# TRIQS/maxent

Hardware: AMD Instinct MI355X
Metric: alpha-solves/s (higher is better)
Workload: dtype f64; 1 GPU; cfg4: ElementwiseMaxEnt 16x16 G(tau) = 256 alpha scans x 100 alpha = 25600 alpha-solves, n_tau=200 n_omega=500 n_s=56; the one batch sharded over 1 GPU(s), element e on rank e mod N; in_flight=1, step=chain kernel + device line fit, problems_on_rank0=25600, kernel=mxe::chain_kernel_mc<32, 2>, waves_per_chain=4, workgroups=512, lds_bytes=77824

## Files before the change

### maxent_amd/csrc/maxent_hip.hip

```cpp
#include "../../include/maxent_hip.h"
#include "mxe_kernel.hip.h"
#include "mxe_kernel_mc.hip.h"
#include "mxe_kernel_lv.hip.h"
#include "mxe_eval.hip.h"
#include "mxe_plan.h"

#include <algorithm>
#include <chrono>
#include <cmath>
#include <cstdio>
#include <cstdlib>
#include <cstring>
#include <new>
#include <string>
#include <map>
#include <vector>
#include <mutex>
#include <thread>
#include <tuple>

using mxe::KParams;

namespace {

// ... 141 lines not shown
            while ((e = hipEventQuery(g_pinned.ev[j & 1])) == hipErrorNotReady) {}
            if (e == hipSuccess) std::memcpy((char*)dst + j * C, g_pinned.buf[j & 1], len);
        }
    }
    return e;
}

template <typename T> struct DevBuf {
    T* p = nullptr; size_t n = 0;
    size_t bytes = 0;
    hipError_t ensure(size_t count) {
        if (count <= n && p) return hipSuccess;
        const size_t need = std::max<size_t>(count, 1) * sizeof(T);
        if (p && need <= bytes) { n = count; return hipSuccess; }
        if (p) { hipDeviceSynchronize(); release(); }
        size_t got = 0;
        void* q = g_pool.take(need, &got);
        static const bool poison = getenv("MXE_POISON_ALLOC") != nullptr;
        if (q) { p = (T*)q; bytes = got; n = count; if (poison) { hipMemset(p, 0xA5, bytes); hipDeviceSynchronize(); } return hipSuccess; }
        hipError_t e = hipMalloc((void**)&p, need);
        if (e == hipSuccess) { n = count; bytes = need; if (poison) { hipMemset(p, 0xA5, bytes); hipDeviceSynchronize(); } }
        return e;
    }
    void release() { if (p && !g_pool.give(p, bytes)) hipFree(p); p = nullptr; n = 0; bytes = 0; }
};

}

struct mxe_ctx {
    int device = 0, n_cu = 256;
    hipStream_t stream = nullptr;
    hipEvent_t ev0 = nullptr, ev1 = nullptr, ev_mark = nullptr;
    int n_tau = 0, n_omega = 0, n_s = 0, NP = 64, nwp = 0;
    std::vector<double> U, S, V;
    std::vector<DataSet> ds;
    bool ds_dirty = true;
    int n_elem = 0;
    std::vector<int> elem_ds, elem_kind;
    std::vector<double> h_sumD, h_D;
    int n_chain = 0, n_alpha = 0;
    std::vector<int> chain_elem;
    std::vector<int> sub_elem, sub_prob0, sub_len, sub_v0, wg_chains;
    int n_sub = 0, n_wg = 0, mc_na = 0, mc_wgpc = 1, wgpc_auto = 2, n_queue = 0, n_solo = 0;
    std::vector<int> excluded;
    DevBuf<int> dexcluded;
    bool mc_gst = false;
    int lv_mode = 0;
    int mc_wgpc_hint = 1;
    int n_wg2 = 0, wgpc2 = 1;
    DevBuf<int> d2_elem, d2_prob0, d2_len, d2_v0, d2_queue, dcnt1_niter, dcnt1_nevals;
    DevBuf<int> drounds;
    int rounds_n[2] = {0, 0};
    int placement_checked = 0;
    DevBuf<double> dgstate_mc;
    std::vector<int> queue;
    std::vector<int> sub_pre;
    std::vector<int> sub_walk0;
    std::vector<double> walk_alpha;
    bool has_walk = false;
    bool has_pre = false;
    mxe_opts opts;
    bool chains_ready = false, launched = false;
    int last_nw = 0, last_lds = 0;
    std::string last_kernel;
    DevBuf<float> dVf, dVtf;
    DevBuf<double> dsel3;
    std::vector<double> h_sel3;
    double* pre_d = nullptr; int32_t* pre_i = nullptr; bool pre_scaled = false;
    double* pre_rows = nullptr; int pre_first = 0, pre_count = 0; bool pre_index = false;
    double* h_sel3_pinned = nullptr; size_t h_sel3_pinned_n = 0;
    DevBuf<double> dproj_U, dproj_err, dproj_G;
    DevBuf<long long> dproj_off;
    bool proj_ready = false;
    std::vector<double> h_rperp;
    std::vector<long long> elem_roff;
    DevBuf<double> drperp;
    DevBuf<long long> delem_roff;
    bool rperp_dirty = false, roff_ready = false;
    DevBuf<double> dV, dVx, dVt, dc, dcinv, dghat, dcperp, dD, dsumD, dalpha, dv0;
    DevBuf<int> delem_ds, delem_kind, dchain_elem, dsub_prob0, dsub_len, dsub_v0, dwg_chains;
    DevBuf<double> dout_v, dout_pack, dout_pack2, dB, dA, dlogdet;
    DevBuf<int> dparent_elem;
    int result_buffer = 0;
    struct View { double* p = nullptr; } dout_H, dout_chi2, dout_S, dout_Q;
    DevBuf<int> dout_niter, dout_nact;
    struct IView { int* p = nullptr; } dout_conv, dout_nevals;
    DevBuf<long long> dprof;
    DevBuf<int> dqueue, dcounter;
    DevBuf<int> dsub_pre, dsub_init, dsub_walk0;
    DevBuf<double> dwalk_alpha;
    DevBuf<double> dinit_tab;
    DevBuf<double> dgstate;
    DevBuf<int> dfin_budget, dfin_out;
    DevBuf<double> dfin_alpha;
    DevBuf<int> dfin_elem, dfin_prob0, dfin_len, dfin_v0;
    DevBuf<double> dfin_start;
    int sel3_nc = 0;
    int last_finished = 0;
    int last_rungs = 0;
    bool has_init = false;
    DevBuf<double> ev_x, ev_alpha, ev_scal, ev_vecw, ev_vecs, ev_mat;
    DevBuf<int> ev_elem;
    DevBuf<double> pv_d;
    DevBuf<int> pv_i;
    DevBuf<double> ps_d;
    DevBuf<double> rr_d;
    DevBuf<int> rr_i;
    DevBuf<double> er_d;
    DevBuf<int> er_i;
    DevBuf<long long> er_l;
    DevBuf<double> rows_out;
    DevBuf<int> rows_idx;
    double chi2_factor = 1.0;
    struct mxe_comm_state* comm = nullptr;
    std::string hip_err;
};

#define MXE_CATCH_ALL \
    catch (const std::bad_alloc&) { return MXE_ERR_NOMEM; } \
    catch (...) { return MXE_ERR_ARG; }

#define HIPCHK(ctx, call) do { hipError_t e__ = (call); if (e__ != hipSuccess) { \
    (ctx)->hip_err = std::string(#call) + ": " + hipGetErrorString(e__); return MXE_ERR_HIP; } } while (0)

namespace {

void jacobi_svd(std::vector<double>& C, int m, int n, std::vector<double>& Q)
{
    Q.assign((size_t)n * n, 0.0);
    for (int i = 0; i < n; ++i) Q[(size_t)i * n + i] = 1.0;
    const double eps = 2.220446049250313e-16;
    for (int sweep = 0; sweep < 60; ++sweep) {
        bool rotated = false;
        for (int p = 0; p < n - 1; ++p) {
            for (int q = p + 1; q < n; ++q) {
                double a = 0.0, b = 0.0, g = 0.0;
                for (int i = 0; i < m; ++i) {
                    const double x = C[(size_t)i * n + p], y = C[(size_t)i * n + q];
                    a += x * x; b += y * y; g += x * y;
                }
                if (a == 0.0 || b == 0.0) continue;
                if (std::fabs(g) <= eps * std::sqrt(a * b)) continue;
                rotated = true;
                const double zeta = (b - a) / (2.0 * g);
                const double t = (zeta >= 0 ? 1.0 : -1.0) /
                                 (std::fabs(zeta) + std::sqrt(1.0 + zeta * zeta));
                const double cs = 1.0 / std::sqrt(1.0 + t * t), sn = cs * t;
                for (int i = 0; i < m; ++i) {
                    const double x = C[(size_t)i * n + p], y = C[(size_t)i * n + q];
                    C[(size_t)i * n + p] = cs * x - sn * y;
                    C[(size_t)i * n + q] = sn * x + cs * y;
                }
                for (int i = 0; i < n; ++i) {
                    const double x = Q[(size_t)i * n + p], y = Q[(size_t)i * n + q];
                    Q[(size_t)i * n + p] = cs * x - sn * y;
                    Q[(size_t)i * n + q] = sn * x + cs * y;
                }
            }
        }
        if (!rotated) break;
    }
}

int build_dataset(mxe_ctx* ctx, int n_rows, const double* U_rot, const double* err, DataSet& d)
{
    const int ns = ctx->n_s;
// ... 588 lines not shown
int g_placement[MXE_MAX_DEVICES];
std::mutex g_placement_mu;

int placement_rule_holds(mxe_ctx* ctx, int n_cu, bool* holds)
{
    *holds = false;
    if (getenv("MXE_FORCE_NO_SOLO_RULE")) return MXE_OK;
    const int dev = ctx->device;
    if (dev < 0 || dev >= MXE_MAX_DEVICES) return MXE_OK;
    std::lock_guard<std::mutex> lk(g_placement_mu);
    if (g_placement[dev] == 0) {
        const int n = 2 * n_cu;
        DevBuf<unsigned> d;
        HIPCHK(ctx, d.ensure((size_t)2 * n));
        HIPCHK(ctx, hipFuncSetAttribute((const void*)placement_probe_kernel, hipFuncAttributeMaxDynamicSharedMemorySize, 73728));
        std::vector<unsigned> h((size_t)2 * n);
        bool ok = true;
        for (int rep = 0; rep < 2 && ok; ++rep) {
            hipLaunchKernelGGL(placement_probe_kernel, dim3(n), dim3(256), 73728, ctx->stream, d.p);
            HIPCHK(ctx, hipGetLastError());
            HIPCHK(ctx, hipMemcpyAsync(h.data(), d.p, h.size() * 4, hipMemcpyDeviceToHost, ctx->stream));
            HIPCHK(ctx, stream_wait(ctx->stream));
            for (int b = 0; b < n_cu && ok; ++b)
                ok = ((h[2 * b] >> 8) & 0xff) == ((h[2 * (b + n_cu)] >> 8) & 0xff) && (h[2 * b + 1] & 0xf) == (h[2 * (b + n_cu) + 1] & 0xf);
        }
        d.release();
        g_placement[dev] = ok ? 1 : 2;
    }
    *holds = g_placement[dev] == 1;
    return MXE_OK;
}

void read_plan_env(mxe::PlanEnv& env)
{
    if (const char* e = getenv("MXE_TAPER")) env.taper = std::max(0.2, atof(e));
    if (const char* e = getenv("MXE_LADDER_RATIO")) env.ladder_ratio = std::max(1.05, atof(e));
    env.no_lds_basis = getenv("MXE_NO_LDS_BASIS") != nullptr; env.no_split_by_kind = getenv("MXE_NO_SPLIT_BY_KIND") != nullptr;
    env.no_ladder = getenv("MXE_NO_LADDER") != nullptr; env.no_na64 = getenv("MXE_NO_NA64") != nullptr; env.no_sorted_static = getenv("MXE_NO_SORTED_STATIC") != nullptr;
}
}

int mxe_chains_upload(mxe_ctx* ctx, int n_chain, int n_alpha,
                      const int32_t* elem_of_chain, const double* alpha_scaled,
                      const double* v0, const mxe_opts* opts)
try {
    if (!ctx || n_chain < 1 || n_alpha < 1 || !elem_of_chain || !alpha_scaled || !v0) return MXE_ERR_ARG;
    if (ctx->n_elem < 1) return MXE_ERR_STATE;
    HIPCHK(ctx, hipSetDevice(ctx->device));
    if (ctx->ds_dirty) { int rc = upload_bases(ctx); if (rc != MXE_OK) return rc; }
    const int ns = ctx->n_s, NP = ctx->NP, nw = ctx->n_omega, nwp = ctx->nwp;
    const size_t P = (size_t)n_chain * n_alpha;
    mxe_opts o; if (opts) o = *opts; else mxe_opts_default(&o);
    if (o.maxiter < 1 || o.step_max <= 0 || o.mu_first <= 0 || o.mu_grow <= 1.0 || o.decouple_tol < 0) return MXE_ERR_ARG;
    if (o.waves_per_chain != 0 && o.waves_per_chain != 1 && o.waves_per_chain != 2 && o.waves_per_chain != 4 && o.waves_per_chain != 8) return MXE_ERR_ARG;
    if (o.chains_per_wg != 0 && o.chains_per_wg != 1 && o.chains_per_wg != 4) return MXE_ERR_ARG;
    if (o.alpha_split < 0 || o.wg_per_cu < 0 || o.wg_per_cu > 2 || o.in_flight < 0 || o.in_flight > 64) return MXE_ERR_ARG;
    if (o.precision != MXE_PRECISION_F64 && o.precision != MXE_PRECISION_F32) return MXE_ERR_ARG;
    if (o.precision == MXE_PRECISION_F32 && NP != 64) return MXE_ERR_LIMIT;
    if (!(o.chi2_factor > 0.0) || !std::isfinite(o.chi2_factor)) return MXE_ERR_ARG;
    for (int c = 0; c < n_chain; ++c) if (elem_of_chain[c] < 0 || elem_of_chain[c] >= ctx->n_elem) return MXE_ERR_ARG;
    for (size_t i = 0; i < P; ++i) if (!(alpha_scaled[i] > 0.0) || !std::isfinite(alpha_scaled[i])) return MXE_ERR_ARG;
    std::vector<double> hv0((size_t)n_chain * NP, 0.0);
    for (int c = 0; c < n_chain; ++c) {
        const DataSet& DS = ctx->ds[ctx->elem_ds[elem_of_chain[c]]];
        for (int k = 0; k < ns; ++k) {
            double s = DS.identity_q ? v0[(size_t)c * ns + k] : 0.0;
            if (!DS.identity_q) for (int j = 0; j < ns; ++j) s += DS.Q[(size_t)j * ns + k] * v0[(size_t)c * ns + j];
            hv0[(size_t)c * NP + k] = s;
        }
    }
    std::vector<double> alpha_dev(alpha_scaled, alpha_scaled + P);
    if (o.chi2_factor != 1.0) for (double& a : alpha_dev) a /= o.chi2_factor;
    std::vector<int> ds_rows(ctx->ds.size()); std::vector<double> ds_c32(ctx->ds.size(), 0.0);
    for (size_t d = 0; d < ctx->ds.size(); ++d) { ds_rows[d] = ctx->ds[d].n_rows; if (ns > 32) ds_c32[d] = ctx->ds[d].c[32]; }
    mxe::PlanInput in;
    in.n_chain = n_chain; in.n_alpha = n_alpha; in.elem_of_chain = elem_of_chain; in.alpha = alpha_dev.data();
    in.elem_kind = ctx->elem_kind.data(); in.elem_ds = ctx->elem_ds.data(); in.elem_sumD = ctx->h_sumD.data();
    in.n_ds = (int)ctx->ds.size(); in.ds_rows = ds_rows.data(); in.ds_c32 = ds_c32.data();
    in.n_s = ns; in.NP = NP; in.n_omega_pad = nwp; in.n_cu = ctx->n_cu; in.opts = o;
    in.lds_lv = mxe::lv_lds_bytes(ns, nwp) + mxe::LV_STATIC_LDS; in.lds_mc64x1 = mc_lds_bytes(64, nwp, 1);
    in.lds_mc32x1 = mc_lds_bytes(32, nwp, 1); in.lds_mc32x2 = mc_lds_bytes(32, nwp, 2);
    in.wgpc_auto = ctx->wgpc_auto; in.mc_wgpc_hint = ctx->mc_wgpc_hint;
    read_plan_env(in.env);
    mxe::LaunchPlan plan;
    if (const int rc = mxe::plan_launch(in, plan); rc != MXE_OK) {
        if (plan.uncovered || plan.covered_twice) fprintf(stderr, "mxe_chains_upload: %zu problems covered by no piece, %zu by two (layout %d, %zu pieces, %zu excluded)\n",
                                                          plan.uncovered, plan.covered_twice, plan.layout, plan.pieces.size(), plan.excluded.size());
        return rc;
    }
    int n_solo = 0, placement_checked = 0;
    if (plan.solo_rule) {
        bool holds = false;
        if (plan.n_solo_wanted > 0) { const int rp = placement_rule_holds(ctx, ctx->n_cu, &holds); if (rp != MXE_OK) return rp; }
        placement_checked = holds ? 1 : 2; n_solo = (holds && plan.lv_mode != 2) ? plan.n_solo_wanted : 0;
    }
    ctx->chains_ready = false; ctx->launched = false; ctx->sel3_nc = 0; ctx->has_init = false;
    ctx->opts = o; ctx->opts.precision = plan.precision; ctx->chi2_factor = o.chi2_factor;
    ctx->n_chain = n_chain; ctx->n_alpha = n_alpha; ctx->chain_elem.assign(elem_of_chain, elem_of_chain + n_chain);
    const size_t n_sub = plan.pieces.size();
    for (auto* v : {&ctx->sub_elem, &ctx->sub_prob0, &ctx->sub_len, &ctx->sub_v0, &ctx->sub_pre, &ctx->sub_walk0}) v->resize(n_sub);
    ctx->n_sub = (int)n_sub; ctx->has_pre = false;
    for (size_t sc = 0; sc < n_sub; ++sc) {
        const mxe::Piece& p = plan.pieces[sc];
        ctx->sub_elem[sc] = p.elem; ctx->sub_prob0[sc] = p.prob0; ctx->sub_len[sc] = p.len; ctx->sub_v0[sc] = p.v0;
        ctx->sub_pre[sc] = p.pre; ctx->sub_walk0[sc] = p.walk0; ctx->has_pre |= p.pre > 0;
    }
    ctx->has_walk = !plan.walk_alpha.empty(); ctx->walk_alpha = std::move(plan.walk_alpha); ctx->excluded = std::move(plan.excluded);
    ctx->queue = std::move(plan.queue); ctx->wg_chains = std::move(plan.wg_chains); ctx->n_queue = (int)ctx->queue.size();
    ctx->mc_na = plan.mc_na; ctx->mc_wgpc = plan.mc_wgpc; ctx->mc_gst = plan.mc_gst; ctx->lv_mode = plan.lv_mode;
    ctx->wgpc_auto = plan.wgpc_auto; ctx->mc_wgpc_hint = plan.mc_wgpc_hint; ctx->n_wg = plan.n_wg; ctx->n_wg2 = plan.n_wg2; ctx->wgpc2 = plan.wgpc2;
    ctx->n_solo = n_solo; ctx->placement_checked = placement_checked;
    auto put = [&](auto& buf, const auto& vec) -> hipError_t {
        if (const hipError_t e = buf.ensure(vec.size()); e != hipSuccess || vec.empty()) return e;
        return hipMemcpyAsync(buf.p, vec.data(), vec.size() * sizeof(vec[0]), hipMemcpyHostToDevice, ctx->stream);
    };
    HIPCHK(ctx, ctx->dcounter.ensure(2)); HIPCHK(ctx, put(ctx->dqueue, ctx->queue)); HIPCHK(ctx, put(ctx->dwg_chains, ctx->wg_chains));
    HIPCHK(ctx, put(ctx->dchain_elem, ctx->sub_elem)); HIPCHK(ctx, put(ctx->dsub_prob0, ctx->sub_prob0));
    HIPCHK(ctx, put(ctx->dsub_len, ctx->sub_len)); HIPCHK(ctx, put(ctx->dsub_v0, ctx->sub_v0));
    HIPCHK(ctx, ctx->dsub_pre.ensure(n_sub));
    if (ctx->has_pre || ctx->mc_gst) HIPCHK(ctx, put(ctx->dsub_pre, ctx->sub_pre));
    if (ctx->has_walk && ctx->has_pre) { HIPCHK(ctx, put(ctx->dsub_walk0, ctx->sub_walk0)); HIPCHK(ctx, put(ctx->dwalk_alpha, ctx->walk_alpha)); }
    if (!ctx->excluded.empty()) HIPCHK(ctx, put(ctx->dexcluded, ctx->excluded));
    HIPCHK(ctx, put(ctx->dalpha, alpha_dev)); HIPCHK(ctx, put(ctx->dv0, hv0)); HIPCHK(ctx, ctx->dout_v.ensure(P * NP));
    HIPCHK(ctx, ctx->dout_pack.ensure(P * nw + 3 * P + (size_t)n_chain * (nw + 1)));
    ctx->result_buffer = 0;
    ctx->dout_H.p = ctx->dout_pack.p; ctx->dout_chi2.p = ctx->dout_pack.p + P * nw;
    ctx->dout_S.p = ctx->dout_chi2.p + P; ctx->dout_Q.p = ctx->dout_S.p + P;
    HIPCHK(ctx, ctx->dout_niter.ensure(3 * P)); HIPCHK(ctx, ctx->dout_nact.ensure(P));
    ctx->dout_conv.p = ctx->dout_niter.p + P; ctx->dout_nevals.p = ctx->dout_conv.p + P;
    std::vector<int> e2, p2, l2;
    if (ctx->lv_mode == 2) {
        e2.resize(P); p2.resize(P); l2.assign(P, 1);
        for (size_t i = 0; i < P; ++i) { e2[i] = elem_of_chain[i / n_alpha]; p2[i] = (int)i; }
        HIPCHK(ctx, put(ctx->d2_elem, e2)); HIPCHK(ctx, put(ctx->d2_len, l2));
        HIPCHK(ctx, put(ctx->d2_prob0, p2)); HIPCHK(ctx, put(ctx->d2_v0, p2)); HIPCHK(ctx, put(ctx->d2_queue, p2));
        HIPCHK(ctx, ctx->dcnt1_niter.ensure(P)); HIPCHK(ctx, ctx->dcnt1_nevals.ensure(P));
    }
    HIPCHK(ctx, stream_wait(ctx->stream));
    { const int rc_init = build_init_table(ctx, n_chain, elem_of_chain, hv0); if (rc_init != MXE_OK) return rc_init; }
    ctx->chains_ready = true;
    return MXE_OK;
}
MXE_CATCH_ALL

constexpr int MC_MAXITER = 32;
static void fill_kparams(mxe_ctx* ctx, KParams& kp)
{
    const mxe_opts& o = ctx->opts;
    kp.n_omega = ctx->n_omega; kp.n_omega_pad = ctx->nwp; kp.n_s = ctx->n_s; kp.NP = ctx->NP;
    kp.n_alpha = ctx->n_alpha; kp.n_chain = ctx->n_chain;
    kp.Vf = ctx->dVf.p; kp.Vtf = ctx->dVtf.p;
    kp.V = ctx->dV.p; kp.Vx = ctx->dVx.p; kp.Vt = ctx->dVt.p; kp.c = ctx->dc.p; kp.cinv = ctx->dcinv.p;
    kp.elem_ds = ctx->delem_ds.p; kp.elem_kind = ctx->delem_kind.p;
    kp.ghat = ctx->dghat.p; kp.cperp = ctx->dcperp.p; kp.D = ctx->dD.p; kp.sumD = ctx->dsumD.p;
    kp.chain_elem = ctx->dchain_elem.p; kp.alpha = ctx->dalpha.p; kp.v0 = ctx->dv0.p;
    kp.chain_prob0 = ctx->dsub_prob0.p; kp.chain_len = ctx->dsub_len.p; kp.chain_v0 = ctx->dsub_v0.p;
    kp.chain_lead = ((ctx->has_pre || ctx->mc_gst) && ctx->mc_na > 0) ? ctx->dsub_pre.p : nullptr;
    const bool walks = ctx->has_walk && ctx->has_pre && ctx->mc_na > 0;
    kp.chain_walk0 = walks ? ctx->dsub_walk0.p : nullptr;
    kp.walk_alpha = walks ? ctx->dwalk_alpha.p : nullptr;
    kp.init_tab = (ctx->has_init && ctx->mc_na > 0) ? ctx->dinit_tab.p : nullptr;
    kp.chain_init = ctx->dsub_init.p;
    kp.n_chain = ctx->n_sub;
    kp.out_v = ctx->dout_v.p; kp.out_H = ctx->dout_H.p; kp.out_chi2 = ctx->dout_chi2.p;
    kp.out_S = ctx->dout_S.p; kp.out_Q = ctx->dout_Q.p; kp.out_niter = ctx->dout_niter.p;
    kp.out_conv = ctx->dout_conv.p; kp.out_nevals = ctx->dout_nevals.p;
    kp.maxiter = o.maxiter; kp.miniter = o.miniter;
    kp.tol_h = o.tol_h; kp.tol_d = o.tol_d; kp.tol_relq = o.tol_relq; kp.stop_estimate = o.stop_estimate != 0;
    kp.step_max = o.step_max; kp.mu_first = o.mu_first; kp.mu_grow = o.mu_grow; kp.mu_max = o.mu_max;
    kp.theta = o.decouple_tol; kp.out_nact = ctx->dout_nact.p;
    kp.prof = nullptr;
    kp.gstate = nullptr;
    kp.mc_maxiter = std::min(o.maxiter, std::max(MC_MAXITER, o.miniter + 8));
    kp.mc_abandon = 1;
    { const char* e = getenv("MXE_MC_MAXEVALS"); kp.mc_maxevals = e ? atoi(e) : 3 * kp.mc_maxiter; }
    kp.prob_maxiter = nullptr;
    kp.out_index = nullptr;
    kp.dbg_hist = nullptr;
    { const char* e = getenv("MXE_STUCK_SKIP"); kp.stuck_skip = e ? atoi(e) : 1; }
}

namespace {
__global__ __launch_bounds__(256)
void clear_excluded_kernel(const int* __restrict__ idx, int n_alpha, int n_omega, int NP, const double* __restrict__ v0,
                           double* __restrict__ H, double* __restrict__ chi2, double* __restrict__ S, double* __restrict__ Q,
                           double* __restrict__ v, int* __restrict__ niter, int* __restrict__ conv, int* __restrict__ nevals, int* __restrict__ nact)
{
    const size_t pidx = (size_t)idx[blockIdx.x];
    const double nan = __builtin_nan("");
    for (int i = threadIdx.x; i < n_omega; i += blockDim.x) H[pidx * n_omega + i] = nan;
    const size_t chain = pidx / n_alpha;
    for (int k = threadIdx.x; k < NP; k += blockDim.x) v[pidx * NP + k] = v0[chain * NP + k];
    if (threadIdx.x == 0) { chi2[pidx] = nan; S[pidx] = nan; Q[pidx] = nan; niter[pidx] = 0; conv[pidx] = 0; nevals[pidx] = 0; nact[pidx] = 0; }
}
__global__ __launch_bounds__(256)
void add_counts_kernel(int* __restrict__ niter, int* __restrict__ nevals, const int* __restrict__ niter1, const int* __restrict__ nevals1, int n)
{
    const int i = blockIdx.x * 256 + threadIdx.x;
    if (i < n) { niter[i] += niter1[i]; nevals[i] += nevals1[i]; }
}
}

namespace {
__global__ __launch_bounds__(256)
void scribble_lds_kernel(unsigned long long pattern, int words, unsigned long long* sink)
{
    extern __shared__ unsigned long long sl[];
    for (int i = threadIdx.x; i < words; i += 256) sl[i] = pattern ? (0x3ff0000000000000ull | ((pattern + (unsigned long long)i * 0x9E3779B97F4A7C15ull) & 0x000fffffffffffffull)) : 0x7ff8000000000000ull;
    __syncthreads();
    if (sink && sl[(threadIdx.x * 7) % words] == 1) sink[0] = 1;
    __builtin_amdgcn_s_sleep(64);
}
hipError_t scribble_lds(hipStream_t s)
{
    static const int mode = getenv("MXE_POISON_LDS") ? atoi(getenv("MXE_POISON_LDS")) : 0;
    if (!mode) return hipSuccess;
    static unsigned long long launches = 0;
    const int bytes = 160 * 1024;
    hipError_t e = hipFuncSetAttribute((const void*)scribble_lds_kernel, hipFuncAttributeMaxDynamicSharedMemorySize, bytes);
    if (e != hipSuccess) return e;
    ++launches;
    const unsigned long long pat = mode == 1 ? 0ull : (launches * 0x2545F4914F6CDD1Dull | 1ull);
    hipLaunchKernelGGL(scribble_lds_kernel, dim3(512), dim3(256), bytes, s, pat, bytes / 8, (unsigned long long*)nullptr);
    return hipGetLastError();
}
}

constexpr double LV_TOL1 = 1e-5;

int mxe_chains_launch(mxe_ctx* ctx)
try {
    if (!ctx) return MXE_ERR_ARG;
    if (!ctx->chains_ready) return MXE_ERR_STATE;
    HIPCHK(ctx, hipSetDevice(ctx->device));
    ctx->pre_d = nullptr; ctx->pre_i = nullptr; ctx->pre_rows = nullptr; ctx->pre_index = false;
    const mxe_opts& o = ctx->opts;
    KParams kp;
    fill_kparams(ctx, kp);
    HIPCHK(ctx, scribble_lds(ctx->stream));
    if (getenv("MXE_COUNT_ROUNDS") && ctx->mc_na > 0 && kp.chain_lead == nullptr && ctx->lv_mode == 0) {
        HIPCHK(ctx, hipMemsetAsync(ctx->dsub_pre.p, 0, (size_t)std::max(ctx->n_sub, 1) * sizeof(int), ctx->stream));
        kp.chain_lead = ctx->dsub_pre.p;
    }
#ifdef MXE_PROFILE
    HIPCHK(ctx, ctx->dprof.ensure(((size_t)ctx->n_sub + 8 * 1024) * 8));
    HIPCHK(ctx, hipMemsetAsync(ctx->dprof.p, 0, ((size_t)ctx->n_sub + 8 * 1024) * 64, ctx->stream));
    kp.prof = ctx->dprof.p;
#endif
    hipError_t e;
    if (ctx->mc_na > 0) {
        if (ctx->lv_mode != 0) {
            const size_t lds1 = mxe::lv_lds_bytes(ctx->n_s, ctx->nwp);
            mxe::MCExtra ex; ex.wg_chains = ctx->dwg_chains.p; ex.n_wg = ctx->n_wg;
            ex.gstate = nullptr; ex.gstate_stride = 0; ex.stagger = 0; ex.n_solo = 0;
            ex.queue = ctx->dqueue.p; ex.n_queue = ctx->n_queue; ex.counter = ctx->dcounter.p;
            HIPCHK(ctx, hipMemsetAsync(ctx->dcounter.p, 0, 2 * sizeof(int), ctx->stream));
            ctx->rounds_n[0] = ctx->n_wg; ctx->rounds_n[1] = (ctx->lv_mode == 2) ? ctx->n_wg2 : 0;
            HIPCHK(ctx, ctx->drounds.ensure((size_t)ctx->rounds_n[0] + ctx->rounds_n[1]));
            HIPCHK(ctx, hipMemsetAsync(ctx->drounds.p, 0, ((size_t)ctx->rounds_n[0] + ctx->rounds_n[1]) * sizeof(int), ctx->stream));
            if (ex.n_queue > 0) ex.wg_chains = ctx->drounds.p;
            else ctx->rounds_n[0] = 0;
            KParams k1 = kp;
            if (ctx->lv_mode == 2) {
                k1.tol_h = std::max(kp.tol_h, LV_TOL1);
                k1.out_H = nullptr;
                k1.out_niter = ctx->dcnt1_niter.p; k1.out_nevals = ctx->dcnt1_nevals.p;
            }
            ctx->last_nw = mxe::LV_NWV; ctx->last_lds = (int)lds1;
            ctx->last_kernel = "mxe::chain_kernel_lv";
            HIPCHK(ctx, hipEventRecord(ctx->ev0, ctx->stream));
            e = hipFuncSetAttribute((const void*)mxe::chain_kernel_lv, hipFuncAttributeMaxDynamicSharedMemorySize, (int)lds1);
            HIPCHK(ctx, e);
            hipLaunchKernelGGL(mxe::chain_kernel_lv, dim3(ctx->n_wg), dim3(64 * mxe::LV_NWV), lds1, ctx->stream, k1, ex);
            HIPCHK(ctx, hipGetLastError());
            if (ctx->lv_mode == 2) {
                const size_t Pn = (size_t)ctx->n_chain * ctx->n_alpha;
                const int W2 = ctx->wgpc2;
                const int NWV2 = (W2 == 1 && ctx->nwp % 256 == 0 && mc_lds_bytes(32, ctx->nwp, 1, 8) <= 160 * 1024 - 6144) ? 8 : 4;
                const size_t lds = mc_lds_bytes(32, ctx->nwp, W2, NWV2);
                if (lds > 160 * 1024 - 6144) return MXE_ERR_LIMIT;
                KParams k2 = kp;
                k2.chain_elem = ctx->d2_elem.p; k2.chain_prob0 = ctx->d2_prob0.p; k2.chain_len = ctx->d2_len.p;
                k2.chain_v0 = ctx->d2_v0.p; k2.v0 = ctx->dout_v.p;
                k2.chain_lead = nullptr; k2.init_tab = nullptr; k2.chain_init = nullptr; k2.chain_walk0 = nullptr; k2.walk_alpha = nullptr;
                k2.n_chain = (int)Pn;
                k2.prof = nullptr;
                mxe::MCExtra e2 = ex;
                e2.n_wg = ctx->n_wg2;
                e2.queue = ctx->d2_queue.p; e2.n_queue = (int)Pn; e2.counter = ctx->dcounter.p + 1;
                e2.wg_chains = ctx->drounds.p + ctx->rounds_n[0];
#define MXE_LAUNCH_MC2(WG_, NWV_) do { \
                e = hipFuncSetAttribute((const void*)mxe::chain_kernel_mc<32, WG_, false, NWV_>, hipFuncAttributeMaxDynamicSharedMemorySize, (int)lds); \
                if (e == hipSuccess) { hipLaunchKernelGGL((mxe::chain_kernel_mc<32, WG_, false, NWV_>), dim3(ctx->n_wg2), dim3(64 * NWV_), lds, ctx->stream, k2, e2); e = hipGetLastError(); } } while (0)
                if (W2 == 2) MXE_LAUNCH_MC2(2, 4); else if (NWV2 == 8) MXE_LAUNCH_MC2(1, 8); else MXE_LAUNCH_MC2(1, 4);
#undef MXE_LAUNCH_MC2
                HIPCHK(ctx, e);
                hipLaunchKernelGGL(add_counts_kernel, dim3((unsigned)((Pn + 255) / 256)), dim3(256), 0, ctx->stream,
                                   ctx->dout_niter.p, ctx->dout_nevals.p, ctx->dcnt1_niter.p, ctx->dcnt1_nevals.p, (int)Pn);
                HIPCHK(ctx, hipGetLastError());
                ctx->last_kernel += " + mxe::chain_kernel_mc<32, " + std::to_string(W2) + (NWV2 == 8 ? ", 8 waves>" : ">") + " per alpha";
            }
            HIPCHK(ctx, hipEventRecord(ctx->ev1, ctx->stream));
            ctx->launched = true;
            return MXE_OK;
        }
        const int NA = ctx->mc_na, WGPC = ctx->mc_wgpc;
        const bool GST = ctx->mc_gst;
        const int NWV = (NA == 32 && WGPC == 1 && ctx->nwp % 256 == 0 && o.waves_per_chain != 4 &&
                         mc_lds_bytes(NA, ctx->nwp, 1, 8, GST) <= 160 * 1024 - 6144) ? 8 : 4;
        const size_t lds = mc_lds_bytes(NA, ctx->nwp, WGPC, NWV, GST);
        if (lds > 160 * 1024 - 6144) return MXE_ERR_LIMIT;
        mxe::MCExtra ex; ex.wg_chains = ctx->dwg_chains.p; ex.n_wg = ctx->n_wg;
        ex.gstate = nullptr; ex.gstate_stride = 0;
        if (GST) {
            ex.gstate_stride = mxe::mc_gstate_doubles(ctx->nwp);
            HIPCHK(ctx, ctx->dgstate_mc.ensure((size_t)ctx->n_wg * ex.gstate_stride + 4096));
            ex.gstate = ctx->dgstate_mc.p;
        }
        ex.queue = ctx->dqueue.p; ex.n_queue = ctx->n_queue; ex.counter = ctx->dcounter.p;
        ctx->rounds_n[0] = ctx->rounds_n[1] = 0;
        if (ex.n_queue > 0 && (kp.chain_lead != nullptr || WGPC == 1 || getenv("MXE_COUNT_ROUNDS"))) {
            ctx->rounds_n[0] = ctx->n_wg;
            HIPCHK(ctx, ctx->drounds.ensure((size_t)ctx->n_wg));
            HIPCHK(ctx, hipMemsetAsync(ctx->drounds.p, 0, (size_t)ctx->n_wg * sizeof(int), ctx->stream));
            ex.wg_chains = ctx->drounds.p;
        }
        ex.stagger = 0;
        ex.n_solo = 0;
        int counter0 = 0;
        if (ex.n_queue > 0 && WGPC == 2 && ctx->n_solo > 0) {
            ex.n_solo = ctx->n_solo;
            counter0 = (ctx->n_wg - ex.n_solo) * 4;
        }
        HIPCHK(ctx, hipMemsetD32Async((hipDeviceptr_t)ctx->dcounter.p, counter0, 1, ctx->stream));
        if (!ctx->excluded.empty()) {
            hipLaunchKernelGGL(clear_excluded_kernel, dim3((unsigned)ctx->excluded.size()), dim3(256), 0, ctx->stream,
                               ctx->dexcluded.p, ctx->n_alpha, ctx->n_omega, ctx->NP, ctx->dv0.p, ctx->dout_H.p, ctx->dout_chi2.p,
                               ctx->dout_S.p, ctx->dout_Q.p, ctx->dout_v.p, ctx->dout_niter.p, ctx->dout_conv.p,
                               ctx->dout_nevals.p, ctx->dout_nact.p);
            HIPCHK(ctx, hipGetLastError());
        }
        ctx->last_nw = NWV; ctx->last_lds = (int)lds;
        const bool lead = kp.chain_lead != nullptr;
        ctx->last_kernel = "mxe::chain_kernel_mc<" + std::to_string(NA) + ", " + std::to_string(WGPC) + (lead ? ", lead" : "") +
                           (NWV == 8 ? ", 8 waves" : "") + (GST ? ", device-memory state>" : ">");
        HIPCHK(ctx, hipEventRecord(ctx->ev0, ctx->stream));
#define MXE_LAUNCH_MC(NA_, WG_, LD_, ...) do { constexpr int NWV_ = std::get<0>(std::make_tuple(__VA_ARGS__)); \
        e = hipFuncSetAttribute((const void*)mxe::chain_kernel_mc<NA_, WG_, LD_, __VA_ARGS__>, hipFuncAttributeMaxDynamicSharedMemorySize, (int)lds); \
        if (e == hipSuccess && getenv("MXE_DEBUG_OCC")) { int nb__ = 0; \
            hipOccupancyMaxActiveBlocksPerMultiprocessor(&nb__, (const void*)mxe::chain_kernel_mc<NA_, WG_, LD_, __VA_ARGS__>, 64 * NWV_, lds); \
            fprintf(stderr, "[mxe] lock-step kernel NA=%d NWV=%d lds=%zu: %d workgroup(s) per CU resident\n", NA_, NWV_, (size_t)lds, nb__); } \
        if (e == hipSuccess) { hipLaunchKernelGGL((mxe::chain_kernel_mc<NA_, WG_, LD_, __VA_ARGS__>), dim3(ctx->n_wg), dim3(64 * NWV_), lds, ctx->stream, kp, ex); e = hipGetLastError(); } } while (0)
        if (NA == 64) { if (lead) MXE_LAUNCH_MC(64, 1, true, 4); else MXE_LAUNCH_MC(64, 1, false, 4); }
        else if (GST) { if (NWV == 8) MXE_LAUNCH_MC(32, 1, true, 8, true); else MXE_LAUNCH_MC(32, 1, true, 4, true); }
        else if (NA == 32 && WGPC == 2) { if (lead) MXE_LAUNCH_MC(32, 2, true, 4); else MXE_LAUNCH_MC(32, 2, false, 4); }
        else if (NWV == 8) { if (lead) MXE_LAUNCH_MC(32, 1, true, 8); else MXE_LAUNCH_MC(32, 1, false, 8); }
        else { if (lead) MXE_LAUNCH_MC(32, 1, true, 4); else MXE_LAUNCH_MC(32, 1, false, 4); }
#undef MXE_LAUNCH_MC
        HIPCHK(ctx, e);
    } else {
        ctx->rounds_n[0] = ctx->rounds_n[1] = 0;
        int NW = std::min(o.waves_per_chain, 4);
        if (NW == 0) {
            const int nc = ctx->n_sub;
            NW = (nc >= 2048) ? 1 : (nc >= 1024) ? 2 : 4;
        }
        const bool f32 = (o.precision == MXE_PRECISION_F32);
        size_t lds = lds_bytes(ctx->NP, ctx->nwp, NW, f32);
        while (lds > 160 * 1024 && NW > 1) { NW /= 2; lds = lds_bytes(ctx->NP, ctx->nwp, NW, f32); }
        const bool gst = lds > 160 * 1024;
        if (gst) {
            NW = (ctx->NP == 64) ? 4 : 1;
            lds = lds_bytes(ctx->NP, ctx->nwp, NW, f32, true);
            if (lds > 160 * 1024) return MXE_ERR_LIMIT;
            HIPCHK(ctx, ctx->dgstate.ensure((size_t)ctx->n_sub * 5 * ctx->nwp));
            kp.gstate = ctx->dgstate.p;
        }
        ctx->last_nw = NW; ctx->last_lds = (int)lds;
        ctx->last_kernel = "mxe::chain_kernel<" + std::to_string(NW) + ", " + std::to_string(ctx->NP / 32) + (f32 ? ", float" : ", double") + (gst ? ", device-memory state>" : ">");
        HIPCHK(ctx, hipEventRecord(ctx->ev0, ctx->stream));
        if (gst) {
            if (f32) e = launch_t<4, 2, float, true>(kp, lds, ctx->stream);
            else e = (ctx->NP == 64) ? launch_t<4, 2, double, true>(kp, lds, ctx->stream) : launch_t<1, 4, double, true>(kp, lds, ctx->stream);
        } else
        if (f32) {
            switch (NW) {
                case 1: e = launch_t<1, 2, float>(kp, lds, ctx->stream); break;
                case 2: e = launch_t<2, 2, float>(kp, lds, ctx->stream); break;
                case 4: e = launch_t<4, 2, float>(kp, lds, ctx->stream); break;
                default: e = launch_t<4, 2, float>(kp, lds, ctx->stream); break;
            }
        } else
        switch (NW) {
            case 1: e = launch_nab<1>(ctx->NP, kp, lds, ctx->stream); break;
            case 2: e = launch_nab<2>(ctx->NP, kp, lds, ctx->stream); break;
            case 4: e = launch_nab<4>(ctx->NP, kp, lds, ctx->stream); break;
            default: e = launch_nab<4>(ctx->NP, kp, lds, ctx->stream); break;
        }
        HIPCHK(ctx, e);
    }
    HIPCHK(ctx, hipEventRecord(ctx->ev1, ctx->stream));
    ctx->launched = true;
    return MXE_OK;
}
MXE_CATCH_ALL

int mxe_sync(mxe_ctx* ctx)
{
    if (!ctx) return MXE_ERR_ARG;
    HIPCHK(ctx, hipSetDevice(ctx->device));
    HIPCHK(ctx, stream_wait(ctx->stream));
    return MXE_OK;
}

int mxe_chains_finish(mxe_ctx* ctx, int32_t* n_resolved)
try {
    if (n_resolved) *n_resolved = 0;
    if (!ctx) return MXE_ERR_ARG;
    if (!ctx->launched) return MXE_ERR_STATE;
    ctx->last_finished = 0;
    if (ctx->mc_na == 0) return MXE_OK;
    HIPCHK(ctx, hipSetDevice(ctx->device));
    HIPCHK(ctx, stream_wait(ctx->stream));
    const mxe_opts& o = ctx->opts;
    const size_t P = (size_t)ctx->n_chain * ctx->n_alpha;
    std::vector<int> conv(P), nit(P), nev(P);
    HIPCHK(ctx, hipMemcpy(conv.data(), ctx->dout_conv.p, P * sizeof(int), hipMemcpyDeviceToHost));
    std::vector<int> todo;
    for (size_t i = 0; i < P; ++i) if (!conv[i]) todo.push_back((int)i);
    if (todo.empty()) return MXE_OK;
    HIPCHK(ctx, hipMemcpy(nit.data(), ctx->dout_niter.p, P * sizeof(int), hipMemcpyDeviceToHost));
    HIPCHK(ctx, hipMemcpy(nev.data(), ctx->dout_nevals.p, P * sizeof(int), hipMemcpyDeviceToHost));
    std::vector<char> open(P, 0);
    int n = 0;
    for (int i : todo) if (nit[i] < o.maxiter) { open[i] = 1; ++n; }
    if (n == 0) return MXE_OK;
    ctx->pre_d = nullptr; ctx->pre_i = nullptr; ctx->pre_rows = nullptr; ctx->pre_index = false;
    const int NP = ctx->NP, na = ctx->n_alpha;
    std::vector<int> f_elem, f_prob0, f_len, f_v0;
    std::vector<size_t> f_src;
    constexpr double FIN_COARSE = 1.6;
    const double FIN_RATIO = getenv("MXE_FIN_RATIO") ? std::max(1.05, atof(getenv("MXE_FIN_RATIO"))) : 1.3;
    const int FIN_RUNG_ITERS = getenv("MXE_FIN_RUNG_ITERS") ? std::max(1, atoi(getenv("MXE_FIN_RUNG_ITERS"))) : 10;
    constexpr int FIN_RUNGS_MAX = 40;
    const bool rungs_ok = !getenv("MXE_NO_FINISH_LADDER");
    std::vector<double> halpha(P);
    HIPCHK(ctx, hipMemcpy(halpha.data(), ctx->dalpha.p, P * sizeof(double), hipMemcpyDeviceToHost));
    std::vector<double> e_alpha;
    std::vector<int> e_out, e_budget;
    int n_rungs = 0;
    for (int c = 0; c < ctx->n_chain; ++c)
        for (int i = 0; i < na; ) {
            if (!open[(size_t)c * na + i]) { ++i; continue; }
            int j = i;
            while (j < na && open[(size_t)c * na + j]) ++j;
            f_elem.push_back(ctx->chain_elem[c]); f_prob0.push_back((int)e_alpha.size());
            f_v0.push_back((int)f_v0.size());
            const size_t p_head = (size_t)c * na + i;
            f_src.push_back(i > 0 ? p_head - 1 : ((nit[p_head] > 0 || nev[p_head] > 0) ? p_head : (size_t)-1 - (size_t)c));
            if (rungs_ok && i == 0 && f_src.back() > (size_t)-1 - (size_t)ctx->n_chain - 1) {
                const double a_to = halpha[p_head];
                const double a_from = 0.25 * ctx->ds[ctx->elem_ds[ctx->chain_elem[c]]].n_rows;
                const bool fine_head = na > 1 && std::max(halpha[p_head + 1] / a_to, a_to / halpha[p_head + 1]) <= FIN_COARSE;
                if (fine_head && a_to * FIN_RATIO * FIN_RATIO < a_from) {
                    int m = (int)std::ceil(std::log(a_from / a_to) / std::log(FIN_RATIO) - 1e-9);
                    m = std::max(2, std::min(m, FIN_RUNGS_MAX + 1));
                    const double q = std::pow(a_to / a_from, 1.0 / m);
                    for (int s2 = 0; s2 < m; ++s2) {
                        e_alpha.push_back(a_from * std::pow(q, s2)); e_out.push_back(-1); e_budget.push_back(s2 == 0 ? 3 * FIN_RUNG_ITERS : FIN_RUNG_ITERS);
                        ++n_rungs;
                    }
                }
            }
            for (int k = i; k < j; ++k) {
                const size_t pk = (size_t)c * na + k;
                if (rungs_ok && k > 0) {
                    const double a_from = halpha[pk - 1], a_to = halpha[pk];
                    const double r = a_from > a_to ? a_from / a_to : a_to / a_from;
                    if (r > FIN_COARSE) {
                        int m = (int)std::ceil(std::log(r) / std::log(FIN_RATIO) - 1e-9);
                        m = std::max(2, std::min(m, FIN_RUNGS_MAX + 1));
                        const double q = std::pow(a_to / a_from, 1.0 / m);
                        for (int s2 = 1; s2 < m; ++s2) {
                            e_alpha.push_back(a_from * std::pow(q, s2)); e_out.push_back(-1); e_budget.push_back(FIN_RUNG_ITERS);
                            ++n_rungs;
                        }
                    }
                }
                e_alpha.push_back(halpha[pk]); e_out.push_back((int)pk);
                e_budget.push_back(std::max(1, o.maxiter - nit[pk]));
            }
            f_len.push_back((int)e_alpha.size() - f_prob0.back());
            i = j;
        }
    const int nr = (int)f_elem.size();
    const size_t ne = e_alpha.size();
    HIPCHK(ctx, ctx->dfin_elem.ensure(nr)); HIPCHK(ctx, ctx->dfin_prob0.ensure(nr));
    HIPCHK(ctx, ctx->dfin_len.ensure(nr)); HIPCHK(ctx, ctx->dfin_v0.ensure(nr));
    HIPCHK(ctx, ctx->dfin_start.ensure((size_t)nr * NP));
    HIPCHK(ctx, ctx->dfin_alpha.ensure(ne)); HIPCHK(ctx, ctx->dfin_out.ensure(ne)); HIPCHK(ctx, ctx->dfin_budget.ensure(ne));
    HIPCHK(ctx, hipMemcpyAsync(ctx->dfin_elem.p, f_elem.data(), nr * sizeof(int), hipMemcpyHostToDevice, ctx->stream));
    HIPCHK(ctx, hipMemcpyAsync(ctx->dfin_prob0.p, f_prob0.data(), nr * sizeof(int), hipMemcpyHostToDevice, ctx->stream));
    HIPCHK(ctx, hipMemcpyAsync(ctx->dfin_len.p, f_len.data(), nr * sizeof(int), hipMemcpyHostToDevice, ctx->stream));
    HIPCHK(ctx, hipMemcpyAsync(ctx->dfin_v0.p, f_v0.data(), nr * sizeof(int), hipMemcpyHostToDevice, ctx->stream));
    HIPCHK(ctx, hipMemcpyAsync(ctx->dfin_alpha.p, e_alpha.data(), ne * sizeof(double), hipMemcpyHostToDevice, ctx->stream));
    HIPCHK(ctx, hipMemcpyAsync(ctx->dfin_out.p, e_out.data(), ne * sizeof(int), hipMemcpyHostToDevice, ctx->stream));
    HIPCHK(ctx, hipMemcpyAsync(ctx->dfin_budget.p, e_budget.data(), ne * sizeof(int), hipMemcpyHostToDevice, ctx->stream));
    for (int k = 0; k < nr; ++k) {
        const bool from_v0 = f_src[k] > (size_t)-1 - (size_t)ctx->n_chain - 1;
        const double* from = from_v0 ? ctx->dv0.p + ((size_t)-1 - f_src[k]) * NP : ctx->dout_v.p + f_src[k] * NP;
        HIPCHK(ctx, hipMemcpyAsync(ctx->dfin_start.p + (size_t)k * NP, from, NP * sizeof(double), hipMemcpyDeviceToDevice, ctx->stream));
    }
    HIPCHK(ctx, stream_wait(ctx->stream));
    KParams kp;
    fill_kparams(ctx, kp);
    kp.chain_elem = ctx->dfin_elem.p; kp.chain_prob0 = ctx->dfin_prob0.p; kp.chain_len = ctx->dfin_len.p;
    kp.chain_v0 = ctx->dfin_v0.p; kp.v0 = ctx->dfin_start.p;
    kp.chain_lead = nullptr; kp.init_tab = nullptr; kp.chain_init = nullptr; kp.chain_walk0 = nullptr; kp.walk_alpha = nullptr;
    kp.n_chain = nr;
    kp.alpha = ctx->dfin_alpha.p; kp.out_index = ctx->dfin_out.p; kp.prob_maxiter = ctx->dfin_budget.p;
    ctx->last_rungs = n_rungs;
#ifdef MXE_DEBUG_HIST
    DevBuf<double> dhist;
    if (getenv("MXE_DEBUG_HIST_FILE")) {
        HIPCHK(ctx, dhist.ensure(ne * 48));
        HIPCHK(ctx, hipMemsetAsync(dhist.p, 0, ne * 48 * sizeof(double), ctx->stream));
        kp.dbg_hist = dhist.p;
    }
#endif
#ifdef MXE_PROFILE
    if (ctx->dprof.p && (size_t)nr <= (size_t)ctx->n_sub + 8 * 1024) {
        HIPCHK(ctx, hipMemsetAsync(ctx->dprof.p, 0, ((size_t)ctx->n_sub + 8 * 1024) * 64, ctx->stream));
        kp.prof = ctx->dprof.p;
    }
#endif
    const int NW = 4;
    size_t lds = lds_bytes(NP, ctx->nwp, NW, false);
    hipError_t e;
    HIPCHK(ctx, scribble_lds(ctx->stream));
    if (lds > 160 * 1024) {
        lds = lds_bytes(NP, ctx->nwp, NW, false, true);
        if (lds > 160 * 1024) return MXE_ERR_LIMIT;
        HIPCHK(ctx, ctx->dgstate.ensure((size_t)nr * 5 * ctx->nwp));
        kp.gstate = ctx->dgstate.p;
        e = launch_t<4, 2, double, true>(kp, lds, ctx->stream);
    } else {
        e = launch_t<4, 2>(kp, lds, ctx->stream);
    }
    HIPCHK(ctx, e);
    HIPCHK(ctx, stream_wait(ctx->stream));
#ifdef MXE_DEBUG_HIST
    if (kp.dbg_hist) {
        std::vector<double> hh(ne * 48);
        HIPCHK(ctx, hipMemcpy(hh.data(), dhist.p, ne * 48 * sizeof(double), hipMemcpyDeviceToHost));
        std::vector<int> cv(P);
        HIPCHK(ctx, hipMemcpy(cv.data(), ctx->dout_conv.p, P * sizeof(int), hipMemcpyDeviceToHost));
        std::vector<int> ni(P);
        HIPCHK(ctx, hipMemcpy(ni.data(), ctx->dout_niter.p, P * sizeof(int), hipMemcpyDeviceToHost));
        if (FILE* f = fopen(getenv("MXE_DEBUG_HIST_FILE"), "a")) {
            for (size_t en = 0; en < ne; ++en) {
                if (e_out[en] < 0) continue;
                fprintf(f, "%d %d %d %.6e", e_out[en], cv[e_out[en]], ni[e_out[en]], e_alpha[en]);
                for (int m = 0; m < 48; ++m) fprintf(f, "%s%.3e", (m % 16 == 0) ? " | " : " ", hh[en * 48 + m]);
                fprintf(f, "\n");
            }
            fclose(f);
        }
        dhist.release();
    }
#endif
    std::vector<int> nit2(P), nev2(P);
    HIPCHK(ctx, hipMemcpy(nit2.data(), ctx->dout_niter.p, P * sizeof(int), hipMemcpyDeviceToHost));
    HIPCHK(ctx, hipMemcpy(nev2.data(), ctx->dout_nevals.p, P * sizeof(int), hipMemcpyDeviceToHost));
    for (size_t i = 0; i < P; ++i) if (open[i]) { nit2[i] += nit[i]; nev2[i] += nev[i]; }
    HIPCHK(ctx, hipMemcpy(ctx->dout_niter.p, nit2.data(), P * sizeof(int), hipMemcpyHostToDevice));
    HIPCHK(ctx, hipMemcpy(ctx->dout_nevals.p, nev2.data(), P * sizeof(int), hipMemcpyHostToDevice));
    ctx->last_finished = n;
    if (n_resolved) *n_resolved = n;
    return MXE_OK;
}
MXE_CATCH_ALL

int mxe_chains_fetch(mxe_ctx* ctx, double* out_v, double* out_H, double* out_chi2,
                     double* out_S, double* out_Q, int32_t* out_niter,
                     int32_t* out_converged, int32_t* out_nevals)
try {
    if (!ctx) return MXE_ERR_ARG;
    if (!ctx->launched) return MXE_ERR_STATE;
    HIPCHK(ctx, hipSetDevice(ctx->device));
    HIPCHK(ctx, stream_wait(ctx->stream));
    const size_t P = (size_t)ctx->n_chain * ctx->n_alpha;
    const int ns = ctx->n_s, NP = ctx->NP, nw = ctx->n_omega;
    if (out_H) HIPCHK(ctx, d2h_pipelined(out_H, ctx->dout_H.p, P * nw * 8, ctx->stream));
    const bool pre = ctx->pre_d && out_chi2 == ctx->pre_d && out_S == out_chi2 + P && out_Q == out_S + P &&
                     out_niter == ctx->pre_i && out_converged == out_niter + P && out_nevals == out_converged + P;
    if (pre) {}
    else if (out_chi2 && out_S == out_chi2 + P && out_Q == out_S + P)
        HIPCHK(ctx, hipMemcpy(out_chi2, ctx->dout_chi2.p, 3 * P * 8, hipMemcpyDeviceToHost));
    else {
        if (out_chi2) HIPCHK(ctx, hipMemcpy(out_chi2, ctx->dout_chi2.p, P * 8, hipMemcpyDeviceToHost));
        if (out_S) HIPCHK(ctx, hipMemcpy(out_S, ctx->dout_S.p, P * 8, hipMemcpyDeviceToHost));
        if (out_Q) HIPCHK(ctx, hipMemcpy(out_Q, ctx->dout_Q.p, P * 8, hipMemcpyDeviceToHost));
    }
    if (out_Q && ctx->chi2_factor != 1.0 && !(pre && ctx->pre_scaled)) for (size_t i = 0; i < P; ++i) out_Q[i] *= ctx->chi2_factor;
    if (pre) ctx->pre_scaled = true;
    if (pre) {}
    else if (out_niter && out_converged == out_niter + P && out_nevals == out_converged + P)
        HIPCHK(ctx, hipMemcpy(out_niter, ctx->dout_niter.p, 3 * P * 4, hipMemcpyDeviceToHost));
    else {
        if (out_niter) HIPCHK(ctx, hipMemcpy(out_niter, ctx->dout_niter.p, P * 4, hipMemcpyDeviceToHost));
        if (out_converged) HIPCHK(ctx, hipMemcpy(out_converged, ctx->dout_conv.p, P * 4, hipMemcpyDeviceToHost));
        if (out_nevals) HIPCHK(ctx, hipMemcpy(out_nevals, ctx->dout_nevals.p, P * 4, hipMemcpyDeviceToHost));
    }
    if (out_v) {
        std::vector<double> hv(P * NP);
        HIPCHK(ctx, hipMemcpy(hv.data(), ctx->dout_v.p, P * NP * 8, hipMemcpyDeviceToHost));
        for (size_t pidx = 0; pidx < P; ++pidx) {
            const int chain = (int)(pidx / ctx->n_alpha);
            const DataSet& DS = ctx->ds[ctx->elem_ds[ctx->chain_elem[chain]]];
            for (int k = 0; k < ns; ++k) {
                double s;
                if (DS.identity_q) s = hv[pidx * NP + k];
                else {
                    s = 0.0;
                    for (int j = 0; j < ns; ++j) s += DS.Q[(size_t)k * ns + j] * hv[pidx * NP + j];
                }
                out_v[pidx * ns + k] = s;
            }
        }
    }
    return MXE_OK;
}
MXE_CATCH_ALL

namespace {
struct CopySeg { const uint32_t* src; uint32_t* dst; size_t words; };
__global__ __launch_bounds__(256)
void copy_out_kernel(CopySeg a, CopySeg b)
{
    const size_t stride = (size_t)gridDim.x * 256, t0 = (size_t)blockIdx.x * 256 + threadIdx.x;
    for (size_t i = t0; i < a.words; i += stride) a.dst[i] = a.src[i];
    for (size_t i = t0; i < b.words; i += stride) b.dst[i] = b.src[i];
}
hipError_t copy_out(void* dst_a, const void* src_a, size_t bytes_a, void* dst_b, const void* src_b, size_t bytes_b, bool mapped, hipStream_t s)
{
    if (!mapped || (bytes_a & 3) || (bytes_b & 3)) {
        hipError_t e = bytes_a ? hipMemcpyAsync(dst_a, src_a, bytes_a, hipMemcpyDeviceToHost, s) : hipSuccess;
        if (e == hipSuccess && bytes_b) e = hipMemcpyAsync(dst_b, src_b, bytes_b, hipMemcpyDeviceToHost, s);
        return e;
    }
    CopySeg a{(const uint32_t*)src_a, (uint32_t*)dst_a, bytes_a / 4}, b{(const uint32_t*)src_b, (uint32_t*)dst_b, bytes_b / 4};
    const size_t words = std::max(a.words, b.words);
    const int blocks = (int)std::min<size_t>(64, (words + 255) / 256);
    hipLaunchKernelGGL(copy_out_kernel, dim3(std::max(blocks, 1)), dim3(256), 0, s, a, b);
    return hipGetLastError();
}
}

int mxe_chains_prefetch(mxe_ctx* ctx, double* out_chi2_S_Q, int32_t* out_niter_converged_nevals)
try {
    if (!ctx || !out_chi2_S_Q || !out_niter_converged_nevals) return MXE_ERR_ARG;
    if (!ctx->launched) return MXE_ERR_STATE;
    HIPCHK(ctx, hipSetDevice(ctx->device));
    const size_t P = (size_t)ctx->n_chain * ctx->n_alpha;
    ctx->pre_d = nullptr; ctx->pre_i = nullptr;
    const bool mapped = g_host.holds(out_chi2_S_Q, 3 * P * 8) && g_host.holds(out_niter_converged_nevals, 3 * P * 4);
    HIPCHK(ctx, copy_out(out_chi2_S_Q, ctx->dout_chi2.p, 3 * P * 8, out_niter_converged_nevals, ctx->dout_niter.p, 3 * P * 4, mapped, ctx->stream));
    ctx->pre_d = out_chi2_S_Q; ctx->pre_i = out_niter_converged_nevals; ctx->pre_scaled = false;
    return MXE_OK;
}
MXE_CATCH_ALL

int mxe_chains_fetch_nact(mxe_ctx* ctx, int32_t* out_nact)
{
    if (!ctx || !out_nact) return MXE_ERR_ARG;
    if (!ctx->launched) return MXE_ERR_STATE;
    HIPCHK(ctx, hipSetDevice(ctx->device));
    HIPCHK(ctx, stream_wait(ctx->stream));
    const size_t P = (size_t)ctx->n_chain * ctx->n_alpha;
    HIPCHK(ctx, hipMemcpy(out_nact, ctx->dout_nact.p, P * 4, hipMemcpyDeviceToHost));
    return MXE_OK;
}

int mxe_solve_chains(mxe_ctx* ctx, int n_chain, int n_alpha,
                     const int32_t* elem_of_chain, const double* alpha_scaled,
                     const double* v0, const mxe_opts* opts,
                     double* out_v, double* out_H, double* out_chi2,
                     double* out_S, double* out_Q, int32_t* out_niter,
                     int32_t* out_converged, int32_t* out_nevals)
{
    int rc = mxe_chains_upload(ctx, n_chain, n_alpha, elem_of_chain, alpha_scaled, v0, opts);
    if (rc != MXE_OK) return rc;
    rc = mxe_chains_launch(ctx);
    if (rc != MXE_OK) return rc;
    rc = mxe_chains_finish(ctx, nullptr);
    if (rc != MXE_OK) return rc;
    return mxe_chains_fetch(ctx, out_v, out_H, out_chi2, out_S, out_Q, out_niter, out_converged, out_nevals);
}

int mxe_result_device_ptrs(mxe_ctx* ctx, void** d_H, void** d_chi2, void** d_S, void** d_Q,
                           void** d_v, void** d_niter, void** d_converged)
{
    if (!ctx) return MXE_ERR_ARG;
    if (!ctx->chains_ready) return MXE_ERR_STATE;
    if (d_H) *d_H = ctx->dout_H.p;
    if (d_chi2) *d_chi2 = ctx->dout_chi2.p;
    if (d_S) *d_S = ctx->dout_S.p;
    if (d_Q) *d_Q = ctx->dout_Q.p;
    if (d_v) *d_v = ctx->dout_v.p;
    if (d_niter) *d_niter = ctx->dout_niter.p;
    if (d_converged) *d_converged = ctx->dout_conv.p;
    return MXE_OK;
}

int mxe_ns_padded(mxe_ctx* ctx) { return ctx ? ctx->NP : MXE_ERR_ARG; }

int mxe_set_result_buffer(mxe_ctx* ctx, int which)
{
    if (!ctx || (which != 0 && which != 1)) return MXE_ERR_ARG;
    if (!ctx->chains_ready) return MXE_ERR_STATE;
    HIPCHK(ctx, hipSetDevice(ctx->device));
    const size_t P = (size_t)ctx->n_chain * ctx->n_alpha, nw = ctx->n_omega;
    if (which == 1) HIPCHK(ctx, ctx->dout_pack2.ensure(P * nw + 3 * P + (size_t)ctx->n_chain * (nw + 1)));
    double* base = which ? ctx->dout_pack2.p : ctx->dout_pack.p;
    ctx->result_buffer = which;
    ctx->dout_H.p = base; ctx->dout_chi2.p = base + P * nw; ctx->dout_S.p = ctx->dout_chi2.p + P; ctx->dout_Q.p = ctx->dout_S.p + P;
    return MXE_OK;
}

int mxe_last_kernel_ms(mxe_ctx* ctx, float* ms)
{
    if (!ctx || !ms) return MXE_ERR_ARG;
    if (!ctx->launched) return MXE_ERR_STATE;
    HIPCHK(ctx, hipSetDevice(ctx->device));
    HIPCHK(ctx, hipEventSynchronize(ctx->ev1));
    HIPCHK(ctx, hipEventElapsedTime(ms, ctx->ev0, ctx->ev1));
    return MXE_OK;
}

const char* mxe_last_kernel_name(mxe_ctx* ctx) { return ctx ? ctx->last_kernel.c_str() : ""; }

void* mxe_stream(mxe_ctx* ctx) { return ctx ? (void*)ctx->stream : nullptr; }

int mxe_timing_mark(mxe_ctx* ctx)
{
    if (!ctx) return MXE_ERR_ARG;
    HIPCHK(ctx, hipSetDevice(ctx->device));
    HIPCHK(ctx, hipEventRecord(ctx->ev_mark, ctx->stream));
    return MXE_OK;
}

int mxe_ms_since_mark(mxe_ctx* ctx, float* ms)
{
    if (!ctx || !ms) return MXE_ERR_ARG;
    if (!ctx->launched) return MXE_ERR_STATE;
    HIPCHK(ctx, hipSetDevice(ctx->device));
    HIPCHK(ctx, hipEventSynchronize(ctx->ev1));
    HIPCHK(ctx, hipEventElapsedTime(ms, ctx->ev_mark, ctx->ev1));
    return MXE_OK;
}

int mxe_last_launch_info(mxe_ctx* ctx, int* waves_per_chain, int* n_workgroups, int* lds_bytes)
{
    if (!ctx) return MXE_ERR_ARG;
    if (waves_per_chain) *waves_per_chain = ctx->last_nw;
    if (n_workgroups) *n_workgroups = ctx->n_wg;
    if (lds_bytes) *lds_bytes = ctx->last_lds;
    return MXE_OK;
}

int mxe_schedule_info(mxe_ctx* ctx, int* n_solo, int* placement_rule)
{
    if (!ctx) return MXE_ERR_ARG;
    if (n_solo) *n_solo = ctx->n_solo;
    if (placement_rule) *placement_rule = ctx->placement_checked;
    return MXE_OK;
}

int mxe_launch_depth(mxe_ctx* ctx, int32_t* max_rounds, double* mean_rounds)
try {
    if (!ctx || !max_rounds || !mean_rounds) return MXE_ERR_ARG;
    if (!ctx->launched) return MXE_ERR_STATE;
    HIPCHK(ctx, hipSetDevice(ctx->device));
    HIPCHK(ctx, stream_wait(ctx->stream));
    const size_t n = (size_t)ctx->rounds_n[0] + ctx->rounds_n[1];
    std::vector<int> h(n ? n : 1, 0);
    if (n) HIPCHK(ctx, hipMemcpy(h.data(), ctx->drounds.p, n * sizeof(int), hipMemcpyDeviceToHost));
    size_t off = 0;
    for (int k = 0; k < 2; ++k) {
        int mx = 0; double sum = 0.0; int busy = 0;
        for (int i = 0; i < ctx->rounds_n[k]; ++i) { mx = std::max(mx, h[off + i]); sum += h[off + i]; busy += h[off + i] > 0; }
        max_rounds[k] = mx; mean_rounds[k] = busy ? sum / busy : 0.0;
        off += ctx->rounds_n[k];
    }
    return MXE_OK;
}
MXE_CATCH_ALL

}

#ifdef MXE_PROFILE
extern "C" int mxe_prof_fetch(mxe_ctx* ctx, long long* out )
{
    if (!ctx || !out) return MXE_ERR_ARG;
    HIPCHK(ctx, stream_wait(ctx->stream));
    HIPCHK(ctx, hipMemcpy(out, ctx->dprof.p, ((size_t)ctx->n_sub + 8 * 1024) * 64, hipMemcpyDeviceToHost));
    return MXE_OK;
}
#endif

#include "mxe_factor.hip.h"

template <typename... KArgs, typename... Args>
static hipError_t launch_factor_kernel(void (*k4)(KArgs...), void (*k8)(KArgs...), const mxe_ctx* ctx, size_t P, size_t lds,
                                       Args... args)
{
    void (*k)(KArgs...) = ctx->NP == 64 ? k4 : k8;
    hipError_t e = hipFuncSetAttribute((const void*)k, hipFuncAttributeMaxDynamicSharedMemorySize, (int)lds);
    if (e != hipSuccess) return e;
    hipLaunchKernelGGL(k, dim3((unsigned)P), dim3(256), lds, ctx->stream, args...);
    return hipGetLastError();
}

extern "C" int mxe_logdet(mxe_ctx* ctx, double* out_logdet)
try {
    if (!ctx || !out_logdet) return MXE_ERR_ARG;
    if (!ctx->launched) return MXE_ERR_STATE;
    HIPCHK(ctx, hipSetDevice(ctx->device));
    const size_t P = (size_t)ctx->n_chain * ctx->n_alpha;
    HIPCHK(ctx, ctx->dlogdet.ensure(P));
    HIPCHK(ctx, ctx->dparent_elem.ensure(ctx->chain_elem.size()));
    HIPCHK(ctx, hipMemcpyAsync(ctx->dparent_elem.p, ctx->chain_elem.data(), ctx->chain_elem.size() * sizeof(int),
                               hipMemcpyHostToDevice, ctx->stream));
    const size_t lds = mxe::logdet_lds_bytes(ctx->NP, ctx->nwp);
    if (lds > 160 * 1024) return MXE_ERR_LIMIT;
    HIPCHK(ctx, launch_factor_kernel(mxe::logdet_kernel<4>, mxe::logdet_kernel<8>, ctx, P, lds,
                                     ctx->dV.p, ctx->dc.p, ctx->delem_ds.p, ctx->delem_kind.p, ctx->dD.p, ctx->dparent_elem.p,
                                     ctx->dalpha.p, ctx->dout_H.p, ctx->dlogdet.p, ctx->n_alpha, ctx->n_omega, ctx->nwp, ctx->n_s));
    HIPCHK(ctx, hipMemcpyAsync(out_logdet, ctx->dlogdet.p, P * 8, hipMemcpyDeviceToHost, ctx->stream));
    HIPCHK(ctx, stream_wait(ctx->stream));
    return MXE_OK;
}
MXE_CATCH_ALL

namespace {
struct SvdScratch {
    hipStream_t stream = nullptr;
    hipEvent_t e0 = nullptr, e1 = nullptr;
    std::vector<void*> bufs;
    template <typename T> hipError_t alloc(T** p, size_t count) {
        hipError_t e = hipMalloc((void**)p, std::max<size_t>(count, 1) * sizeof(T));
        if (e == hipSuccess) bufs.push_back((void*)*p);
        return e;
    }
    ~SvdScratch() {
        for (void* b : bufs) hipFree(b);
        if (e0) hipEventDestroy(e0);
        if (e1) hipEventDestroy(e1);
        if (stream) hipStreamDestroy(stream);
    }
};
#define SVDCHK(call) do { hipError_t e__ = (call); if (e__ != hipSuccess) { \
    fprintf(stderr, "[mxe] %s: %s\n", #call, hipGetErrorString(e__)); return MXE_ERR_HIP; } } while (0)
}

namespace {
size_t eval_lds_bytes(int NP, int nwp) { return ((size_t)NP * (NP + 1) + 2 * (size_t)nwp + 7 * (size_t)NP + 16) * sizeof(double); }

int launch_eval(mxe_ctx* ctx, const mxe::EvalParams& ep, size_t P)
{
    const size_t lds = eval_lds_bytes(ctx->NP, ctx->nwp);
    if (lds > 160 * 1024) return MXE_ERR_LIMIT;
    hipError_t e;
#define MXE_LAUNCH_EVAL(NT_) do { \
        e = hipFuncSetAttribute((const void*)mxe::eval_kernel<NT_>, hipFuncAttributeMaxDynamicSharedMemorySize, (int)lds); \
        if (e == hipSuccess) { hipLaunchKernelGGL((mxe::eval_kernel<NT_>), dim3((unsigned)P), dim3(256), lds, ctx->stream, ep); \
                               e = hipGetLastError(); } } while (0)
    if (ctx->NP == 64) MXE_LAUNCH_EVAL(4); else MXE_LAUNCH_EVAL(8);
#undef MXE_LAUNCH_EVAL
    HIPCHK(ctx, e);
    return MXE_OK;
}

void eval_params_base(mxe_ctx* ctx, mxe::EvalParams& ep)
{
    std::memset(&ep, 0, sizeof(ep));
    ep.nw = ctx->n_omega; ep.nwp = ctx->nwp; ep.ns = ctx->n_s; ep.NP = ctx->NP;
    ep.V = ctx->dV.p; ep.Vt = ctx->dVt.p; ep.c = ctx->dc.p;
    ep.elem_ds = ctx->delem_ds.p; ep.elem_kind = ctx->delem_kind.p;
    ep.ghat = ctx->dghat.p; ep.cperp = ctx->dcperp.p; ep.D = ctx->dD.p;
    ep.eta = 1.0; ep.elem_div = 1;
}
}

extern "C" int mxe_eval_batch(mxe_ctx* ctx, int P, const int32_t* elem_of_problem, const double* alpha_scaled,
                              const double* x, int input_is_H, double chi2_factor,
                              double* out_Q, double* out_chi2, double* out_S,
                              double* out_H, double* out_u, double* out_w, double* out_q,
                              double* out_h, double* out_g, double* out_W, double* out_W2)
try {
    if (!ctx || P < 1 || !elem_of_problem || !alpha_scaled || !x) return MXE_ERR_ARG;
    if (ctx->n_elem < 1) return MXE_ERR_STATE;
    if (!(chi2_factor > 0.0) || !std::isfinite(chi2_factor)) return MXE_ERR_ARG;
    HIPCHK(ctx, hipSetDevice(ctx->device));
    if (ctx->ds_dirty) { int rc = upload_bases(ctx); if (rc != MXE_OK) return rc; }
    const int ns = ctx->n_s, NP = ctx->NP, nw = ctx->n_omega;
    const size_t xs = input_is_H ? (size_t)nw : (size_t)NP;
    std::vector<double> hx((size_t)P * xs, 0.0);
    for (int p = 0; p < P; ++p) {
        const int e = elem_of_problem[p];
        if (e < 0 || e >= ctx->n_elem) return MXE_ERR_ARG;
        if (!(alpha_scaled[p] >= 0.0) || !std::isfinite(alpha_scaled[p])) return MXE_ERR_ARG;
        if (input_is_H) { std::copy(x + (size_t)p * nw, x + (size_t)(p + 1) * nw, hx.begin() + (size_t)p * nw); continue; }
// ... 44 lines not shown
    HIPCHK(ctx, stream_wait(ctx->stream));
    std::vector<double> tmp((size_t)ns * ns);
    for (int p = 0; p < P; ++p) {
        const DataSet& DS = ctx->ds[ctx->elem_ds[elem_of_problem[p]]];
        auto vec_out = [&](const std::vector<double>& src, double* dst) {
            for (int k = 0; k < ns; ++k) {
                double s;
                if (DS.identity_q) s = src[(size_t)p * NP + k];
                else { s = 0.0; for (int j = 0; j < ns; ++j) s += DS.Q[(size_t)k * ns + j] * src[(size_t)p * NP + j]; }
                dst[(size_t)p * ns + k] = s;
            }
        };
        auto mat_out = [&](const std::vector<double>& src, double* dst) {
            const double* Xp = src.data() + (size_t)p * NP * NP;
            double* out = dst + (size_t)p * ns * ns;
            if (DS.identity_q) {
                for (int i = 0; i < ns; ++i) for (int j = 0; j < ns; ++j) out[(size_t)i * ns + j] = Xp[(size_t)i * NP + j];
                return;
            }
            for (int i = 0; i < ns; ++i) for (int j = 0; j < ns; ++j) {
                double s = 0.0;
                for (int k = 0; k < ns; ++k) s += Xp[(size_t)i * NP + k] * DS.Q[(size_t)j * ns + k];
                tmp[(size_t)i * ns + j] = s;
            }
            for (int i = 0; i < ns; ++i) for (int j = 0; j < ns; ++j) {
                double s = 0.0;
                for (int k = 0; k < ns; ++k) s += DS.Q[(size_t)i * ns + k] * tmp[(size_t)k * ns + j];
                out[(size_t)i * ns + j] = s;
            }
        };
        if (out_h) vec_out(hh, out_h);
        if (out_g) vec_out(hg, out_g);
        if (wantW) mat_out(hW, out_W);
        if (wantW2) mat_out(hW2, out_W2);
    }
    return MXE_OK;
}
MXE_CATCH_ALL

#include "mxe_postvar.hip.h"
#include "mxe_postsample.hip.h"

namespace {
struct PostStage {
    size_t lds = 0;
    std::vector<double> ha;
    std::vector<int> hi;
};

int stage_posterior(mxe_ctx* ctx, int P, const int32_t* elem_of_problem, const double* alpha_scaled, const double* H,
                    const int32_t* problem_index, double chi2_factor, size_t n_max, const double* z, size_t n_z, PostStage& st)
{
    if (ctx->n_elem < 1) return MXE_ERR_STATE;
    if (!H && !ctx->launched) return MXE_ERR_STATE;
    if (!(chi2_factor > 0.0) || !std::isfinite(chi2_factor)) return MXE_ERR_ARG;
    if (n_max > 0x7fffffffull) return MXE_ERR_ARG;
    st.lds = mxe::postvar_lds_bytes(ctx->NP, ctx->nwp);
    if (st.lds > 160 * 1024) return MXE_ERR_LIMIT;
    if (z) for (size_t i = 0; i < n_z; ++i) if (!std::isfinite(z[i])) return MXE_ERR_ARG;
    HIPCHK(ctx, hipSetDevice(ctx->device));
    if (ctx->ds_dirty) { int rc = upload_bases(ctx); if (rc != MXE_OK) return rc; }
    const size_t n_last = (size_t)ctx->n_chain * ctx->n_alpha;
    st.ha.resize(P);
    st.hi.resize((size_t)2 * P);
    for (int p = 0; p < P; ++p) {
        const int e = elem_of_problem[p];
        if (e < 0 || e >= ctx->n_elem) return MXE_ERR_ARG;
        if (!(alpha_scaled[p] > 0.0) || !std::isfinite(alpha_scaled[p])) return MXE_ERR_ARG;
        st.ha[p] = alpha_scaled[p] / chi2_factor;
        st.hi[p] = e;
        int row = p;
        if (!H) {
            row = problem_index ? problem_index[p] : p;
            if (row < 0 || (size_t)row >= n_last) return MXE_ERR_ARG;
        }
        st.hi[(size_t)P + p] = row;
    }
    return MXE_OK;
}

int upload_posterior(mxe_ctx* ctx, const PostStage& st, int P, const double* H, double* d, size_t oH, mxe::FactorParams& fp)
{
    const int nw = ctx->n_omega;
    HIPCHK(ctx, ctx->pv_i.ensure((size_t)2 * P));
    HIPCHK(ctx, hipMemcpyAsync(d, st.ha.data(), (size_t)P * 8, hipMemcpyHostToDevice, ctx->stream));
    if (H) HIPCHK(ctx, hipMemcpyAsync(d + oH, H, (size_t)P * nw * 8, hipMemcpyHostToDevice, ctx->stream));
    HIPCHK(ctx, hipMemcpyAsync(ctx->pv_i.p, st.hi.data(), st.hi.size() * sizeof(int), hipMemcpyHostToDevice, ctx->stream));
    fp.V = ctx->dV.p; fp.c = ctx->dc.p; fp.elem_ds = ctx->delem_ds.p; fp.elem_kind = ctx->delem_kind.p; fp.D = ctx->dD.p;
    fp.elem = ctx->pv_i.p; fp.alpha = d;
    fp.H = H ? d + oH : ctx->dout_H.p; fp.row = H ? nullptr : ctx->pv_i.p + P;
    fp.nw = nw; fp.nwp = ctx->nwp; fp.ns = ctx->n_s;
    return MXE_OK;
}
}

extern "C" int mxe_posterior_var(mxe_ctx* ctx, int P, const int32_t* elem_of_problem, const double* alpha_scaled,
                                 const double* H, const int32_t* problem_index, double chi2_factor,
                                 int n_f, const double* F, double* out_var, double* out_diag, double* out_prior,
                                 float* out_ms)
try {
    if (!ctx || P < 1 || !elem_of_problem || !alpha_scaled || n_f < 0 || (n_f > 0 && (!F || !out_var))) return MXE_ERR_ARG;
    if (n_f == 0 && !out_diag) return MXE_ERR_ARG;
    if (out_prior && n_f == 0) return MXE_ERR_ARG;
    const int nw = ctx->n_omega;
    PostStage st;
    const size_t n_max = std::max({(size_t)P * (size_t)std::max(n_f, 1), (size_t)P * nw, (size_t)n_f * nw});
    int rc = stage_posterior(ctx, P, elem_of_problem, alpha_scaled, H, problem_index, chi2_factor, n_max, nullptr, 0, st);
    if (rc != MXE_OK) return rc;
    for (size_t i = 0; i < (size_t)n_f * nw; ++i) if (!std::isfinite(F[i])) return MXE_ERR_ARG;
    const size_t oH = (size_t)P, oF = oH + (H ? (size_t)P * nw : 0), oV = oF + (size_t)n_f * nw, oP = oV + (size_t)P * n_f,
                 oD = oP + (out_prior ? (size_t)P * n_f : 0), total = oD + (out_diag ? (size_t)P * nw : 0);
    HIPCHK(ctx, ctx->pv_d.ensure(total));
    double* d = ctx->pv_d.p;
    mxe::PostVarParams pp;
    rc = upload_posterior(ctx, st, P, H, d, oH, pp);
    if (rc != MXE_OK) return rc;
    if (n_f) HIPCHK(ctx, hipMemcpyAsync(d + oF, F, (size_t)n_f * nw * 8, hipMemcpyHostToDevice, ctx->stream));
    pp.F = n_f ? d + oF : nullptr;
    pp.out_var = d + oV; pp.out_prior = out_prior ? d + oP : nullptr; pp.out_diag = out_diag ? d + oD : nullptr;
    pp.n_f = n_f;
    SvdScratch sc;
    if (out_ms) {
        HIPCHK(ctx, hipEventCreate(&sc.e0)); HIPCHK(ctx, hipEventCreate(&sc.e1));
        HIPCHK(ctx, hipEventRecord(sc.e0, ctx->stream));
    }
    HIPCHK(ctx, launch_factor_kernel(mxe::postvar_kernel<4>, mxe::postvar_kernel<8>, ctx, (size_t)P, st.lds, pp));
    if (out_ms) HIPCHK(ctx, hipEventRecord(sc.e1, ctx->stream));
    if (n_f) HIPCHK(ctx, hipMemcpyAsync(out_var, d + oV, (size_t)P * n_f * 8, hipMemcpyDeviceToHost, ctx->stream));
    if (out_prior) HIPCHK(ctx, hipMemcpyAsync(out_prior, d + oP, (size_t)P * n_f * 8, hipMemcpyDeviceToHost, ctx->stream));
    if (out_diag) HIPCHK(ctx, hipMemcpyAsync(out_diag, d + oD, (size_t)P * nw * 8, hipMemcpyDeviceToHost, ctx->stream));
    HIPCHK(ctx, stream_wait(ctx->stream));
    if (out_ms) HIPCHK(ctx, hipEventElapsedTime(out_ms, sc.e0, sc.e1));
    if (chi2_factor != 1.0) {
        for (size_t i = 0; i < (size_t)P * n_f; ++i) { out_var[i] /= chi2_factor; if (out_prior) out_prior[i] /= chi2_factor; }
        if (out_diag) for (size_t i = 0; i < (size_t)P * nw; ++i) out_diag[i] /= chi2_factor;
    }
    return MXE_OK;
}
MXE_CATCH_ALL

extern "C" int mxe_posterior_sample(mxe_ctx* ctx, int P, const int32_t* elem_of_problem, const double* alpha_scaled,
                                    const double* H, const int32_t* problem_index, double chi2_factor,
                                    int n_samples, uint64_t seed, const uint64_t* stream, const double* z,
                                    double* out_dH, float* out_ms)
try {
    if (!ctx || P < 1 || !elem_of_problem || !alpha_scaled || !out_dH || n_samples < 1 || (!z && !stream)) return MXE_ERR_ARG;
    const int nw = ctx->n_omega, nz = nw + ctx->n_s;
    const size_t n_z = (size_t)P * n_samples * nz, n_out = (size_t)P * n_samples * nw;
    PostStage st;
    int rc = stage_posterior(ctx, P, elem_of_problem, alpha_scaled, H, problem_index, chi2_factor, n_z, z, n_z, st);
    if (rc != MXE_OK) return rc;
    const size_t oS = (size_t)P, oH = oS + (size_t)P, oZ = oH + (H ? (size_t)P * nw : 0), oO = oZ + n_z, total = oO + n_out;
    HIPCHK(ctx, ctx->ps_d.ensure(total));
    double* d = ctx->ps_d.p;
    mxe::PostSampleParams pp;
    rc = upload_posterior(ctx, st, P, H, d, oH, pp);
    if (rc != MXE_OK) return rc;
    if (z) HIPCHK(ctx, hipMemcpyAsync(d + oZ, z, n_z * 8, hipMemcpyHostToDevice, ctx->stream));
    else HIPCHK(ctx, hipMemcpyAsync(d + oS, stream, (size_t)P * 8, hipMemcpyHostToDevice, ctx->stream));
    pp.z = d + oZ; pp.out = d + oO; pp.scale = 1.0 / std::sqrt(chi2_factor);
    pp.n_samples = n_samples;
    SvdScratch sc;
    if (out_ms) {
        HIPCHK(ctx, hipEventCreate(&sc.e0)); HIPCHK(ctx, hipEventCreate(&sc.e1));
        HIPCHK(ctx, hipEventRecord(sc.e0, ctx->stream));
    }
// ... 112 lines not shown
MXE_CATCH_ALL

extern "C" int mxe_normals(int device, uint64_t seed, uint64_t stream, int n_samples, int n, double* out_z)
try {
    if (n_samples < 1 || n < 1 || !out_z || (size_t)n_samples * (size_t)n > 0x7fffffffull) return MXE_ERR_ARG;
    int ndev = 0;
    if (hipGetDeviceCount(&ndev) != hipSuccess || ndev < 1) return MXE_ERR_NODEVICE;
    if (device < 0 || device >= ndev) return MXE_ERR_ARG;
    SvdScratch sc;
    SVDCHK(hipSetDevice(device));
    SVDCHK(hipStreamCreateWithFlags(&sc.stream, hipStreamNonBlocking));
    double* dz;
    SVDCHK(sc.alloc(&dz, (size_t)n_samples * n));
    const size_t per = (size_t)n_samples * ((n + 1) / 2);
    hipLaunchKernelGGL(mxe::normals_kernel, dim3((unsigned)std::min<size_t>((per + 255) / 256, 1024), 1), dim3(256), 0, sc.stream,
                       seed, (const uint64_t*)nullptr, stream, 1, n_samples, n, dz);
    SVDCHK(hipGetLastError());
    SVDCHK(hipMemcpyAsync(out_z, dz, (size_t)n_samples * n * 8, hipMemcpyDeviceToHost, sc.stream));
    SVDCHK(hipStreamSynchronize(sc.stream));
    return MXE_OK;
}
MXE_CATCH_ALL

extern "C" int mxe_entropy(int device, int kind, int n_omega, int P, const double* H, const double* D,
                           double* out_S, double* out_dS, double* out_ddS)
try {
    if (n_omega < 1 || P < 1 || !H || !D || (kind != MXE_ENTROPY_NORMAL && kind != MXE_ENTROPY_PLUSMINUS)) return MXE_ERR_ARG;
    int ndev = 0;
    if (hipGetDeviceCount(&ndev) != hipSuccess || ndev < 1) return MXE_ERR_NODEVICE;
    if (device < 0 || device >= ndev) return MXE_ERR_ARG;
    SvdScratch sc;
    SVDCHK(hipSetDevice(device));
    SVDCHK(hipStreamCreateWithFlags(&sc.stream, hipStreamNonBlocking));
    const size_t n = n_omega;
    double *dH, *dD, *dS, *dd, *ddd;
    SVDCHK(sc.alloc(&dH, (size_t)P * n)); SVDCHK(sc.alloc(&dD, n)); SVDCHK(sc.alloc(&dS, (size_t)P));
    SVDCHK(sc.alloc(&dd, (size_t)P * n)); SVDCHK(sc.alloc(&ddd, (size_t)P * n));
    SVDCHK(hipMemcpyAsync(dH, H, (size_t)P * n * 8, hipMemcpyHostToDevice, sc.stream));
    SVDCHK(hipMemcpyAsync(dD, D, n * 8, hipMemcpyHostToDevice, sc.stream));
    hipLaunchKernelGGL(mxe::entropy_kernel, dim3((unsigned)P), dim3(256), 0, sc.stream, kind, n_omega, dH, dD, dS, dd, ddd);
    SVDCHK(hipGetLastError());
    if (out_S) SVDCHK(hipMemcpyAsync(out_S, dS, (size_t)P * 8, hipMemcpyDeviceToHost, sc.stream));
    if (out_dS) SVDCHK(hipMemcpyAsync(out_dS, dd, (size_t)P * n * 8, hipMemcpyDeviceToHost, sc.stream));
    if (out_ddS) SVDCHK(hipMemcpyAsync(out_ddS, ddd, (size_t)P * n * 8, hipMemcpyDeviceToHost, sc.stream));
    SVDCHK(hipStreamSynchronize(sc.stream));
    return MXE_OK;
}
MXE_CATCH_ALL

extern "C" int mxe_audit(mxe_ctx* ctx, double* out_corr, double* out_gmax)
try {
    if (!ctx || (!out_corr && !out_gmax)) return MXE_ERR_ARG;
    if (!ctx->launched) return MXE_ERR_STATE;
    HIPCHK(ctx, hipSetDevice(ctx->device));
    const size_t P = (size_t)ctx->n_chain * ctx->n_alpha;
    HIPCHK(ctx, ctx->ev_scal.ensure(2 * P));
    HIPCHK(ctx, ctx->dparent_elem.ensure(ctx->chain_elem.size()));
    HIPCHK(ctx, hipMemcpyAsync(ctx->dparent_elem.p, ctx->chain_elem.data(), ctx->chain_elem.size() * sizeof(int),
                               hipMemcpyHostToDevice, ctx->stream));
    mxe::EvalParams ep;
    eval_params_base(ctx, ep);
    ep.elem = ctx->dparent_elem.p; ep.elem_div = ctx->n_alpha;
    ep.alpha = ctx->dalpha.p;
    ep.x = ctx->dout_v.p; ep.x_stride = ctx->NP;
    ep.want_audit = 1;
    ep.corr = ctx->ev_scal.p; ep.gmax = ctx->ev_scal.p + P;
    int rc = launch_eval(ctx, ep, P);
    if (rc != MXE_OK) return rc;
    if (out_corr) HIPCHK(ctx, hipMemcpyAsync(out_corr, ep.corr, P * 8, hipMemcpyDeviceToHost, ctx->stream));
    if (out_gmax) HIPCHK(ctx, hipMemcpyAsync(out_gmax, ep.gmax, P * 8, hipMemcpyDeviceToHost, ctx->stream));
    HIPCHK(ctx, stream_wait(ctx->stream));
    return MXE_OK;
}
MXE_CATCH_ALL

extern "C" int mxe_select_launch(mxe_ctx* ctx, int p2_deg)
try {
    if (!ctx || (p2_deg != 0 && p2_deg != 1)) return MXE_ERR_ARG;
    if (!ctx->launched) return MXE_ERR_STATE;
    HIPCHK(ctx, hipSetDevice(ctx->device));
    const size_t P = (size_t)ctx->n_chain * ctx->n_alpha;
    double* sel = ctx->dout_Q.p + P;
    double* idx = sel + (size_t)ctx->n_chain * ctx->n_omega;
    hipLaunchKernelGGL(mxe::linefit_kernel, dim3(ctx->n_chain), dim3(256), ((size_t)11 * ctx->n_alpha + 6 + 28) * sizeof(double), ctx->stream,
                       ctx->dalpha.p, ctx->dout_chi2.p, ctx->dout_H.p, ctx->n_alpha, ctx->n_omega, p2_deg, sel, idx);
    HIPCHK(ctx, hipGetLastError());
    return MXE_OK;
}
MXE_CATCH_ALL

extern "C" int mxe_select3_launch(mxe_ctx* ctx, int p2_deg, double gamma)
try {
    if (!ctx || (p2_deg != 0 && p2_deg != 1) || !(gamma > 0.0)) return MXE_ERR_ARG;
    if (!ctx->launched) return MXE_ERR_STATE;
    HIPCHK(ctx, hipSetDevice(ctx->device));
    const size_t P = (size_t)ctx->n_chain * ctx->n_alpha, nc = ctx->n_chain, nw = ctx->n_omega;
    double* sel = ctx->dout_Q.p + P;
    double* idx = sel + nc * nw;
    HIPCHK(ctx, ctx->dsel3.ensure(3 * nc * (nw + 1)));
    ctx->pre_rows = nullptr; ctx->pre_index = false;
    hipLaunchKernelGGL(mxe::linefit_kernel, dim3(ctx->n_chain), dim3(256), ((size_t)11 * ctx->n_alpha + 6 + 28) * sizeof(double), ctx->stream,
                       ctx->dalpha.p, ctx->dout_chi2.p, ctx->dout_H.p, ctx->n_alpha, ctx->n_omega, p2_deg, sel, idx,
                       ctx->dout_S.p, gamma, ctx->dsel3.p, ctx->dsel3.p + 3 * nc);
    HIPCHK(ctx, hipGetLastError());
    ctx->sel3_nc = ctx->n_chain;
    return MXE_OK;
}
MXE_CATCH_ALL

extern "C" int mxe_select3_fetch_rows(mxe_ctx* ctx, int32_t* out_index , int first, int count,
                                      double* out_H_selected )
try {
    if (!ctx || first < 0 || count < 0 || first + count > 3 || (!out_index && !out_H_selected)) return MXE_ERR_ARG;
    if (!ctx->launched || !ctx->dsel3.p || ctx->sel3_nc != ctx->n_chain) return MXE_ERR_STATE;
    HIPCHK(ctx, hipSetDevice(ctx->device));
    const size_t nc = ctx->n_chain, nw = ctx->n_omega;
    if (ctx->pre_index && ctx->h_sel3_pinned_n >= 3 * nc && (count == 0 || (out_H_selected == ctx->pre_rows && first == ctx->pre_first && count == ctx->pre_count))) {
        HIPCHK(ctx, stream_wait(ctx->stream));
        if (out_index) for (size_t i = 0; i < 3 * nc; ++i) out_index[i] = (int32_t)ctx->h_sel3_pinned[i];
        return MXE_OK;
    }
    if (out_index) {
        ctx->h_sel3.resize(3 * nc);
        HIPCHK(ctx, hipMemcpyAsync(ctx->h_sel3.data(), ctx->dsel3.p, 3 * nc * 8, hipMemcpyDeviceToHost, ctx->stream));
    }
    HIPCHK(ctx, stream_wait(ctx->stream));
    if (out_H_selected && count > 0)
        HIPCHK(ctx, d2h_pipelined(out_H_selected, ctx->dsel3.p + 3 * nc + (size_t)first * nc * nw, (size_t)count * nc * nw * 8, ctx->stream));
    if (out_index) for (size_t i = 0; i < 3 * nc; ++i) out_index[i] = (int32_t)ctx->h_sel3[i];
    return MXE_OK;
}
MXE_CATCH_ALL

extern "C" int mxe_select3_prefetch_rows(mxe_ctx* ctx, int first, int count, double* out_H_selected )
try {
    if (!ctx || first < 0 || count < 0 || first + count > 3 || (count > 0 && !out_H_selected)) return MXE_ERR_ARG;
    if (!ctx->launched || !ctx->dsel3.p || ctx->sel3_nc != ctx->n_chain) return MXE_ERR_STATE;
    HIPCHK(ctx, hipSetDevice(ctx->device));
    const size_t nc = ctx->n_chain, nw = ctx->n_omega;
    ctx->pre_rows = nullptr; ctx->pre_index = false;
    if (ctx->h_sel3_pinned_n < 3 * nc) {
        if (ctx->h_sel3_pinned) { (void)hipHostFree(ctx->h_sel3_pinned); ctx->h_sel3_pinned = nullptr; ctx->h_sel3_pinned_n = 0; }
        HIPCHK(ctx, hipHostMalloc((void**)&ctx->h_sel3_pinned, 3 * nc * 8, hipHostMallocDefault));
        ctx->h_sel3_pinned_n = 3 * nc;
    }
    const size_t row_bytes = (size_t)count * nc * nw * 8;
    const bool mapped = count == 0 || g_host.holds(out_H_selected, row_bytes);
    if (mapped)
        HIPCHK(ctx, copy_out(ctx->h_sel3_pinned, ctx->dsel3.p, 3 * nc * 8, out_H_selected, ctx->dsel3.p + 3 * nc + (size_t)first * nc * nw, row_bytes, true, ctx->stream));
    else {
        HIPCHK(ctx, hipMemcpyAsync(ctx->h_sel3_pinned, ctx->dsel3.p, 3 * nc * 8, hipMemcpyDeviceToHost, ctx->stream));
        HIPCHK(ctx, hipMemcpyAsync(out_H_selected, ctx->dsel3.p + 3 * nc + (size_t)first * nc * nw, row_bytes, hipMemcpyDeviceToHost, ctx->stream));
    }
    ctx->pre_index = true; ctx->pre_rows = count > 0 ? out_H_selected : nullptr; ctx->pre_first = first; ctx->pre_count = count;
    return MXE_OK;
}
MXE_CATCH_ALL

extern "C" int mxe_select3_fetch(mxe_ctx* ctx, int32_t* out_index , double* out_H_selected )
{
    if (!ctx || !out_index) return MXE_ERR_ARG;
    return mxe_select3_fetch_rows(ctx, out_index, 0, out_H_selected ? 3 : 0, out_H_selected);
}

extern "C" int mxe_select_fetch(mxe_ctx* ctx, int32_t* out_index, double* out_H_selected)
try {
    if (!ctx) return MXE_ERR_ARG;
    if (!ctx->launched) return MXE_ERR_STATE;
    HIPCHK(ctx, hipSetDevice(ctx->device));
    const size_t P = (size_t)ctx->n_chain * ctx->n_alpha, nc = ctx->n_chain, nw = ctx->n_omega;
    const double* sel = ctx->dout_Q.p + P;
    HIPCHK(ctx, stream_wait(ctx->stream));
    if (out_H_selected) HIPCHK(ctx, hipMemcpy(out_H_selected, sel, nc * nw * 8, hipMemcpyDeviceToHost));
    if (out_index) {
        std::vector<double> hi(nc);
        HIPCHK(ctx, hipMemcpy(hi.data(), sel + nc * nw, nc * 8, hipMemcpyDeviceToHost));
        for (size_t c = 0; c < nc; ++c) out_index[c] = (int32_t)hi[c];
    }
    return MXE_OK;
}
MXE_CATCH_ALL

namespace {
__global__ __launch_bounds__(256)
void rows_gather_kernel(const double* __restrict__ H, const int* __restrict__ idx, int n_omega, double* __restrict__ out)
{
    const double* src = H + (size_t)idx[blockIdx.x] * n_omega;
    double* dst = out + (size_t)blockIdx.x * n_omega;
    for (int i = threadIdx.x; i < n_omega; i += 256) dst[i] = src[i];
}
}

extern "C" int mxe_fetch_rows(mxe_ctx* ctx, int n_rows, const int32_t* problem_index, double* out_H)
try {
    if (!ctx || n_rows < 1 || !problem_index || !out_H) return MXE_ERR_ARG;
    if (!ctx->launched) return MXE_ERR_STATE;
    HIPCHK(ctx, hipSetDevice(ctx->device));
    const size_t P = (size_t)ctx->n_chain * ctx->n_alpha, nw = ctx->n_omega;
    for (int r = 0; r < n_rows; ++r)
        if (problem_index[r] < 0 || (size_t)problem_index[r] >= P) return MXE_ERR_ARG;
    HIPCHK(ctx, ctx->rows_idx.ensure(n_rows));
    HIPCHK(ctx, ctx->rows_out.ensure((size_t)n_rows * nw));
    HIPCHK(ctx, hipMemcpyAsync(ctx->rows_idx.p, problem_index, (size_t)n_rows * 4, hipMemcpyHostToDevice, ctx->stream));
    hipLaunchKernelGGL(rows_gather_kernel, dim3(n_rows), dim3(256), 0, ctx->stream,
                       (const double*)ctx->dout_H.p, (const int*)ctx->rows_idx.p, (int)nw, ctx->rows_out.p);
    HIPCHK(ctx, hipGetLastError());
    HIPCHK(ctx, hipMemcpyAsync(out_H, ctx->rows_out.p, (size_t)n_rows * nw * 8, hipMemcpyDeviceToHost, ctx->stream));
    HIPCHK(ctx, stream_wait(ctx->stream));
    return MXE_OK;
}
MXE_CATCH_ALL

#include <rccl/rccl.h>
#include <dlfcn.h>
namespace {
struct Rccl {
    void* lib = nullptr;
    ncclResult_t (*GetUniqueId)(ncclUniqueId*) = nullptr;
    ncclResult_t (*CommInitRank)(ncclComm_t*, int, ncclUniqueId, int) = nullptr;
    ncclResult_t (*CommInitAll)(ncclComm_t*, int, const int*) = nullptr;
    ncclResult_t (*CommDestroy)(ncclComm_t) = nullptr;
    ncclResult_t (*Send)(const void*, size_t, ncclDataType_t, int, ncclComm_t, hipStream_t) = nullptr;
    ncclResult_t (*Recv)(void*, size_t, ncclDataType_t, int, ncclComm_t, hipStream_t) = nullptr;
    ncclResult_t (*AllReduce)(const void*, void*, size_t, ncclDataType_t, ncclRedOp_t, ncclComm_t, hipStream_t) = nullptr;
    ncclResult_t (*GroupStart)() = nullptr;
    ncclResult_t (*GroupEnd)() = nullptr;
    const char* (*GetErrorString)(ncclResult_t) = nullptr;
    bool load() {
        if (lib) return true;
        const char* names[] = {"librccl.so.1", "/opt/rocm/lib/librccl.so.1", "librccl.so"};
        for (const char* n : names) { lib = dlopen(n, RTLD_NOW | RTLD_GLOBAL); if (lib) break; }
        if (!lib) return false;
#define MXE_SYM(field, name) field = reinterpret_cast<decltype(field)>(dlsym(lib, name)); if (!field) { dlclose(lib); lib = nullptr; return false; }
        MXE_SYM(GetUniqueId, "ncclGetUniqueId"); MXE_SYM(CommInitRank, "ncclCommInitRank"); MXE_SYM(CommInitAll, "ncclCommInitAll");
        MXE_SYM(CommDestroy, "ncclCommDestroy"); MXE_SYM(Send, "ncclSend"); MXE_SYM(Recv, "ncclRecv");
        MXE_SYM(AllReduce, "ncclAllReduce"); MXE_SYM(GroupStart, "ncclGroupStart"); MXE_SYM(GroupEnd, "ncclGroupEnd"); MXE_SYM(GetErrorString, "ncclGetErrorString");
#undef MXE_SYM
        return true;
    }
};
Rccl g_rccl;
#define NCCLCHK(ctx, call) do { ncclResult_t r__ = (call); if (r__ != ncclSuccess) { \
    (ctx)->hip_err = std::string(#call) + ": " + g_rccl.GetErrorString(r__); return MXE_ERR_HIP; } } while (0)
}

struct mxe_comm_state {
    ncclComm_t comm = nullptr;
    int n_ranks = 1, rank = 0;
    bool copy_transport = false;
    bool loopback = false;
    std::vector<mxe_ctx*> local;
    DevBuf<double> recv;
    DevBuf<double> small;
};

extern "C" int mxe_comm_unique_id(char* out_id128)
{
    if (!out_id128) return MXE_ERR_ARG;
    if (!g_rccl.load()) return MXE_ERR_NODEVICE;
    ncclUniqueId id;
    if (g_rccl.GetUniqueId(&id) != ncclSuccess) return MXE_ERR_HIP;
    std::memcpy(out_id128, id.internal, NCCL_UNIQUE_ID_BYTES);
    return MXE_OK;
}

extern "C" int mxe_comm_init(mxe_ctx* ctx, int n_ranks, int rank, const char* id128)
try {
    if (!ctx || n_ranks < 1 || rank < 0 || rank >= n_ranks || !id128) return MXE_ERR_ARG;
    if (!g_rccl.load()) { ctx->hip_err = "librccl.so.1 could not be loaded"; return MXE_ERR_NODEVICE; }
    HIPCHK(ctx, hipSetDevice(ctx->device));
    comm_release(ctx);
    ctx->comm = new mxe_comm_state();
    ctx->comm->n_ranks = n_ranks; ctx->comm->rank = rank;
    ncclUniqueId id;
    std::memcpy(id.internal, id128, NCCL_UNIQUE_ID_BYTES);
    NCCLCHK(ctx, g_rccl.CommInitRank(&ctx->comm->comm, n_ranks, id, rank));
    return MXE_OK;
}
MXE_CATCH_ALL

extern "C" int mxe_comm_init_local(mxe_ctx** ctxs, int n)
try {
    if (!ctxs || n < 1) return MXE_ERR_ARG;
// ... 24 lines not shown
        ctxs[r]->comm->n_ranks = n; ctxs[r]->comm->rank = r;
        ctxs[r]->comm->comm = comms[r];
        ctxs[r]->comm->copy_transport = !(distinct && n > 1);
        ctxs[r]->comm->local.assign(ctxs, ctxs + n);
    }
    return MXE_OK;
}
MXE_CATCH_ALL

static void comm_release(mxe_ctx* ctx)
{
    if (!ctx || !ctx->comm) return;
    if (ctx->comm->comm && g_rccl.lib) g_rccl.CommDestroy(ctx->comm->comm);
    ctx->comm->recv.release();
    ctx->comm->small.release();
    delete ctx->comm;
    ctx->comm = nullptr;
}

extern "C" int mxe_comm_set_loopback(mxe_ctx* ctx, int on)
{
    if (!ctx) return MXE_ERR_ARG;
    if (!ctx->comm || !ctx->comm->comm || !ctx->comm->local.empty()) return MXE_ERR_STATE;
    ctx->comm->loopback = on != 0;
    return MXE_OK;
}

extern "C" int mxe_comm_destroy(mxe_ctx* ctx)
{
    if (!ctx) return MXE_ERR_ARG;
    hipSetDevice(ctx->device);
    comm_release(ctx);
    return MXE_OK;
}

static void gather_span(mxe_ctx* ctx, int what, double** p, size_t* count)
{
    const size_t P = (size_t)ctx->n_chain * ctx->n_alpha, nw = ctx->n_omega, nc = ctx->n_chain;
    const size_t compact = 3 * P + nc * (nw + 1);
    if (what == MXE_GATHER_FULL) { *p = ctx->dout_H.p; *count = P * nw + compact; }
    else { *p = ctx->dout_chi2.p; *count = compact; }
}

static int gather_enqueue(mxe_ctx* ctx, int root, int what, const int64_t* counts)
{
    mxe_comm_state* cm = ctx->comm;
    double* mine; size_t n_mine;
    gather_span(ctx, what, &mine, &n_mine);
    if ((int64_t)n_mine != counts[cm->rank]) return MXE_ERR_ARG;
    HIPCHK(ctx, hipSetDevice(ctx->device));
    if (cm->rank == root) {
        size_t off = 0;
        for (int r = 0; r < cm->n_ranks; ++r) {
            if (r == root && cm->loopback && !cm->copy_transport) {
                NCCLCHK(ctx, g_rccl.Send(mine, n_mine, ncclDouble, root, cm->comm, ctx->stream));
                NCCLCHK(ctx, g_rccl.Recv(cm->recv.p + off, n_mine, ncclDouble, root, cm->comm, ctx->stream));
            }
            else if (r == root) HIPCHK(ctx, hipMemcpyAsync(cm->recv.p + off, mine, n_mine * 8, hipMemcpyDeviceToDevice, ctx->stream));
            else if (!cm->copy_transport) NCCLCHK(ctx, g_rccl.Recv(cm->recv.p + off, (size_t)counts[r], ncclDouble, r, cm->comm, ctx->stream));
            off += (size_t)counts[r];
        }
    } else if (!cm->copy_transport) {
        NCCLCHK(ctx, g_rccl.Send(mine, n_mine, ncclDouble, root, cm->comm, ctx->stream));
    }
    return MXE_OK;
}

static int gather_reserve(mxe_ctx* root_ctx, int n_ranks, const int64_t* counts)
{
    size_t total = 0;
    for (int r = 0; r < n_ranks; ++r) { if (counts[r] < 0) return MXE_ERR_ARG; total += (size_t)counts[r]; }
    HIPCHK(root_ctx, hipSetDevice(root_ctx->device));
    HIPCHK(root_ctx, root_ctx->comm->recv.ensure(total));
    return MXE_OK;
}

extern "C" int mxe_gather(mxe_ctx* ctx, int root, int what, const int64_t* counts, double* recv_host)
try {
    if (!ctx || !counts || (what != MXE_GATHER_COMPACT && what != MXE_GATHER_FULL)) return MXE_ERR_ARG;
    if (!ctx->comm || !ctx->launched) return MXE_ERR_STATE;
    mxe_comm_state* cm = ctx->comm;
    if (root < 0 || root >= cm->n_ranks) return MXE_ERR_ARG;
    if (!cm->local.empty()) return MXE_ERR_STATE;
    if (cm->rank == root) { const int rr = gather_reserve(ctx, cm->n_ranks, counts); if (rr != MXE_OK) return rr; }
    const bool grouped = cm->n_ranks > 1 || cm->loopback;
    if (grouped) NCCLCHK(ctx, g_rccl.GroupStart());
    const int rc = gather_enqueue(ctx, root, what, counts);
    if (grouped) NCCLCHK(ctx, g_rccl.GroupEnd());
    if (rc != MXE_OK) return rc;
    if (recv_host && cm->rank == root) {
        size_t total = 0;
        for (int r = 0; r < cm->n_ranks; ++r) total += (size_t)counts[r];
        HIPCHK(ctx, hipMemcpyAsync(recv_host, cm->recv.p, total * 8, hipMemcpyDeviceToHost, ctx->stream));
        HIPCHK(ctx, stream_wait(ctx->stream));
    }
    return MXE_OK;
}
MXE_CATCH_ALL

extern "C" int mxe_gather_local(mxe_ctx** ctxs, int n, int root, int what, const int64_t* counts, double* recv_host)
try {
    if (!ctxs || n < 1 || root < 0 || root >= n || !counts || (what != MXE_GATHER_COMPACT && what != MXE_GATHER_FULL)) return MXE_ERR_ARG;
    for (int r = 0; r < n; ++r)
        if (!ctxs[r] || !ctxs[r]->comm || ctxs[r]->comm->n_ranks != n || ctxs[r]->comm->rank != r || !ctxs[r]->launched) return MXE_ERR_STATE;
    mxe_ctx* rt = ctxs[root];
    const bool copy = rt->comm->copy_transport;
    { const int rr = gather_reserve(rt, n, counts); if (rr != MXE_OK) return rr; }
    if (copy) {
        for (int r = 0; r < n; ++r) {
            if (r == root) continue;
            HIPCHK(ctxs[r], hipSetDevice(ctxs[r]->device));
            HIPCHK(ctxs[r], hipEventRecord(ctxs[r]->ev_mark, ctxs[r]->stream));
            HIPCHK(rt, hipSetDevice(rt->device));
            HIPCHK(rt, hipStreamWaitEvent(rt->stream, ctxs[r]->ev_mark, 0));
        }
    } else {
        NCCLCHK(rt, g_rccl.GroupStart());
    }
    int rc = MXE_OK;
    for (int r = 0; r < n && rc == MXE_OK; ++r) rc = gather_enqueue(ctxs[r], root, what, counts);
    if (!copy) NCCLCHK(rt, g_rccl.GroupEnd());
    if (rc != MXE_OK) return rc;
    if (copy) {
        HIPCHK(rt, hipSetDevice(rt->device));
        size_t off = 0;
        for (int r = 0; r < n; ++r) {
            if (r != root) {
                double* src; size_t cnt;
                gather_span(ctxs[r], what, &src, &cnt);
                HIPCHK(rt, hipMemcpyAsync(rt->comm->recv.p + off, src, cnt * 8, hipMemcpyDeviceToDevice, rt->stream));
            }
            off += (size_t)counts[r];
        }
    }
    if (recv_host) {
        size_t total = 0;
        for (int r = 0; r < n; ++r) total += (size_t)counts[r];
        HIPCHK(rt, hipSetDevice(rt->device));
        HIPCHK(rt, hipMemcpyAsync(recv_host, rt->comm->recv.p, total * 8, hipMemcpyDeviceToHost, rt->stream));
        HIPCHK(rt, stream_wait(rt->stream));
    }
    return MXE_OK;
}
MXE_CATCH_ALL

extern "C" int mxe_comm_allreduce(mxe_ctx* ctx, double* inout_host, int n, int op)
try {
    if (!ctx || !inout_host || n < 1 || n > 64 || (op != 0 && op != 1)) return MXE_ERR_ARG;
    if (!ctx->comm) return MXE_ERR_STATE;
    mxe_comm_state* cm = ctx->comm;
    if ((cm->n_ranks == 1 && !cm->loopback) || !cm->local.empty()) return MXE_OK;
    HIPCHK(ctx, hipSetDevice(ctx->device));
    HIPCHK(ctx, cm->small.ensure(64));
    HIPCHK(ctx, hipMemcpyAsync(cm->small.p, inout_host, (size_t)n * 8, hipMemcpyHostToDevice, ctx->stream));
    NCCLCHK(ctx, g_rccl.AllReduce(cm->small.p, cm->small.p, (size_t)n, ncclDouble, op == 0 ? ncclSum : ncclMax, cm->comm, ctx->stream));
    HIPCHK(ctx, hipMemcpyAsync(inout_host, cm->small.p, (size_t)n * 8, hipMemcpyDeviceToHost, ctx->stream));
    HIPCHK(ctx, stream_wait(ctx->stream));
    return MXE_OK;
}
MXE_CATCH_ALL

extern "C" int mxe_shard_plan(int n_elem, int n_ranks, int32_t* rank_of_elem, int32_t* local_index, int32_t* n_local)
{
    if (n_elem < 0 || n_ranks < 1 || !rank_of_elem || !local_index || !n_local) return MXE_ERR_ARG;
    for (int r = 0; r < n_ranks; ++r) n_local[r] = 0;
    for (int e = 0; e < n_elem; ++e) {
        const int r = e % n_ranks;
        rank_of_elem[e] = r;
        local_index[e] = n_local[r]++;
    }
    return MXE_OK;
}

namespace mxe {
__global__ __launch_bounds__(256)
void output_map_kernel(const double* __restrict__ Bt, const double* __restrict__ H,
                       double* __restrict__ A, int nw)
{
    extern __shared__ double hs[];
    const double* Hp = H + (size_t)blockIdx.x * nw;
    for (int k = threadIdx.x; k < nw; k += blockDim.x) hs[k] = Hp[k];
    __syncthreads();
    for (int j = threadIdx.x; j < nw; j += blockDim.x) {
        double a0 = 0.0, a1 = 0.0;
        int k = 0;
        for (; k + 1 < nw; k += 2) {
            a0 = fma(Bt[(size_t)k * nw + j], hs[k], a0);
            a1 = fma(Bt[(size_t)(k + 1) * nw + j], hs[k + 1], a1);
        }
        if (k < nw) a0 = fma(Bt[(size_t)k * nw + j], hs[k], a0);
        A[(size_t)blockIdx.x * nw + j] = a0 + a1;
    }
}
}

extern "C" int mxe_apply_output_map(mxe_ctx* ctx, const double* B, double* out_A)
try {
    if (!ctx || !B || !out_A) return MXE_ERR_ARG;
    if (!ctx->launched) return MXE_ERR_STATE;
    HIPCHK(ctx, hipSetDevice(ctx->device));
    const int nw = ctx->n_omega;
    const size_t P = (size_t)ctx->n_chain * ctx->n_alpha;
    std::vector<double> Bt((size_t)nw * nw);
    for (int j = 0; j < nw; ++j) for (int k = 0; k < nw; ++k) Bt[(size_t)k * nw + j] = B[(size_t)j * nw + k];
    HIPCHK(ctx, ctx->dB.ensure(Bt.size()));
    HIPCHK(ctx, ctx->dA.ensure(P * nw));
    HIPCHK(ctx, hipMemcpyAsync(ctx->dB.p, Bt.data(), Bt.size() * 8, hipMemcpyHostToDevice, ctx->stream));
    hipLaunchKernelGGL(mxe::output_map_kernel, dim3((unsigned)P), dim3(256), (size_t)nw * 8, ctx->stream,
                       ctx->dB.p, ctx->dout_H.p, ctx->dA.p, nw);
    HIPCHK(ctx, hipGetLastError());
    HIPCHK(ctx, hipMemcpyAsync(out_A, ctx->dA.p, P * nw * 8, hipMemcpyDeviceToHost, ctx->stream));
    HIPCHK(ctx, stream_wait(ctx->stream));
    return MXE_OK;
}
MXE_CATCH_ALL

#include "mxe_svd.hip.h"


namespace {
constexpr size_t SVD_LDS_LIMIT = 60 * 1024;
constexpr size_t svd_lds_bytes(int m_rows)
{
    return ((size_t)m_rows + 16 + 8 + mxe::SVD_RCAP + mxe::SVD_RCAP / 2) * sizeof(double);
}

bool svd_args_ok(int n_grid, int n_omega, int n_b, const double* grid, const double* omega, const double* delta,
                 const double* preblur_b, double threshold, int ns_max, const double* out_U, const double* out_S,
                 const double* out_V, const int32_t* out_ns)
{
    return n_grid >= 1 && n_omega >= 1 && n_b >= 1 && grid && omega && delta && preblur_b && out_U && out_S && out_V &&
           out_ns && ns_max >= 1 && ns_max <= mxe::SVD_RCAP && threshold >= 0.0;
}

template <class Kern, class... Args>
void launch_fill(Kern kernel, hipStream_t st, int nel, Args... args)
{
    hipLaunchKernelGGL(kernel, dim3((nel + 255) / 256), dim3(256), 0, st, args...);
}

template <class Fill>
int kernel_svd_common(int device, int n_grid, int m_rows, int n_omega, const double* grid, const double* omega,
                      const double* delta, int n_b, const double* preblur_b, double threshold, int ns_max,
                      double* out_K, double* out_U, double* out_S, double* out_V, int32_t* out_ns,
                      int32_t* out_info, float* out_ms, Fill fill)
{
    int ndev = 0;
    if (hipGetDeviceCount(&ndev) != hipSuccess || ndev < 1) return MXE_ERR_NODEVICE;
    if (device < 0 || device >= ndev) return MXE_ERR_ARG;
    const size_t lds = svd_lds_bytes(m_rows);
    if (lds > SVD_LDS_LIMIT) return MXE_ERR_LIMIT;
    SVDCHK(hipSetDevice(device));
    SvdScratch sc;
    SVDCHK(hipStreamCreateWithFlags(&sc.stream, hipStreamNonBlocking));
    SVDCHK(hipEventCreate(&sc.e0));
    SVDCHK(hipEventCreate(&sc.e1));
    const size_t m = m_rows, n = n_omega, R = mxe::SVD_RCAP;
    double *dgrid, *dom, *ddel, *dKt0, *dr1, *ddc, *dB;
    mxe::SvdParams sp;
    sp.m = m_rows; sp.n = n_omega; sp.ns_max = ns_max; sp.threshold = threshold;
    SVDCHK(sc.alloc(&dgrid, n_grid)); SVDCHK(sc.alloc(&dom, n)); SVDCHK(sc.alloc(&ddel, n));
    SVDCHK(sc.alloc(&dKt0, n * m)); SVDCHK(sc.alloc(&dr1, n)); SVDCHK(sc.alloc(&ddc, n)); SVDCHK(sc.alloc(&dB, n * n));
    SVDCHK(sc.alloc(&sp.A, (size_t)n_b * n * m)); SVDCHK(sc.alloc(&sp.Vh, (size_t)n_b * R * m));
    SVDCHK(sc.alloc(&sp.Rm, (size_t)n_b * R * n)); SVDCHK(sc.alloc(&sp.Jt, (size_t)n_b * R * R));
    SVDCHK(sc.alloc(&sp.Qc, (size_t)n_b * R * m)); SVDCHK(sc.alloc(&sp.cn2, (size_t)n_b * n));
    SVDCHK(sc.alloc(&sp.perm, (size_t)n_b * n));
    SVDCHK(sc.alloc(&sp.out_U, (size_t)n_b * m * ns_max)); SVDCHK(sc.alloc(&sp.out_S, (size_t)n_b * ns_max));
    SVDCHK(sc.alloc(&sp.out_V, (size_t)n_b * n * ns_max)); SVDCHK(sc.alloc(&sp.out_info, (size_t)n_b * 4));
    SVDCHK(hipMemcpyAsync(dgrid, grid, (size_t)n_grid * 8, hipMemcpyHostToDevice, sc.stream));
    SVDCHK(hipMemcpyAsync(dom, omega, n * 8, hipMemcpyHostToDevice, sc.stream));
    SVDCHK(hipMemcpyAsync(ddel, delta, n * 8, hipMemcpyHostToDevice, sc.stream));
    SVDCHK(hipEventRecord(sc.e0, sc.stream));
    fill(sc.stream, dgrid, dom, dKt0);
    SVDCHK(hipGetLastError());
    for (int ib = 0; ib < n_b; ++ib) {
        double* Ai = sp.A + (size_t)ib * n * m;
        const double b = preblur_b[ib];
        if (b > 0.0) {
            hipLaunchKernelGGL(mxe::preblur_rows, dim3(n_omega), dim3(256), 0, sc.stream, dom, ddel, b, n_omega, dr1);
            hipLaunchKernelGGL(mxe::preblur_cols, dim3(n_omega), dim3(256), 0, sc.stream, dom, ddel, b, n_omega, dr1, ddc);
            hipLaunchKernelGGL(mxe::preblur_matrix, dim3((n_omega * n_omega + 255) / 256), dim3(256), 0, sc.stream, dom, b, n_omega, dr1, ddc, dB);
            hipLaunchKernelGGL(mxe::preblur_product, dim3(n_omega), dim3(256), n * 8, sc.stream, dKt0, ddel, dB, m_rows, n_omega, Ai);
            SVDCHK(hipGetLastError());
        } else {
            SVDCHK(hipMemcpyAsync(Ai, dKt0, n * m * 8, hipMemcpyDeviceToDevice, sc.stream));
        }
    }
// ... 295 lines not shown
        for (size_t b = 0; b < m; ++b) {
            const int32_t c = counts[r * m + b];
            if (c < 0) return MXE_ERR_ARG;
            s += c;
        }
        if (s <= 0) return MXE_ERR_ARG;
        hNr[r] = (double)s;
    }
    for (size_t s = 0; s < ns; ++s) if (rank[s] < 0 || rank[s] > n_data) return MXE_ERR_ARG;
    if (!all_finite(bins, nel) || !all_finite(T, ns * n * n)) return MXE_ERR_ARG;
    int ndev = 0;
    if (hipGetDeviceCount(&ndev) != hipSuccess || ndev < 1) return MXE_ERR_NODEVICE;
    if (device < 0 || device >= ndev) return MXE_ERR_ARG;
    SVDCHK(hipSetDevice(device));
    SvdScratch sc;
    SVDCHK(hipStreamCreateWithFlags(&sc.stream, hipStreamNonBlocking));
    mxe::ResampleParams p;
    p.m = n_bins; p.n = n_data; p.n_res = n_res;
    double *dbins, *dNr, *dT;
    int *dcounts, *drank;
    SVDCHK(sc.alloc(&dbins, nel)); SVDCHK(sc.alloc(&dcounts, nr * m)); SVDCHK(sc.alloc(&dNr, nr));
    SVDCHK(sc.alloc(&dT, ns * n * n)); SVDCHK(sc.alloc(&drank, ns));
    SVDCHK(sc.alloc(&p.part, ns * mxe::BINS_NWAVE * n * 2)); SVDCHK(sc.alloc(&p.D, ns * nr * n));
    SVDCHK(sc.alloc(&p.out_mean, ns * n)); SVDCHK(sc.alloc(&p.out_G, ns * nr * n)); SVDCHK(sc.alloc(&p.out_dev, ns * nr * n));
    p.bins = dbins; p.counts = dcounts; p.Nr = dNr; p.T = dT; p.rank = drank;
    SVDCHK(hipMemcpyAsync(dbins, bins, nel * 8, hipMemcpyHostToDevice, sc.stream));
    SVDCHK(hipMemcpyAsync(dcounts, counts, nr * m * 4, hipMemcpyHostToDevice, sc.stream));
    SVDCHK(hipMemcpyAsync(dNr, hNr.data(), nr * 8, hipMemcpyHostToDevice, sc.stream));
    SVDCHK(hipMemcpyAsync(dT, T, ns * n * n * 8, hipMemcpyHostToDevice, sc.stream));
    SVDCHK(hipMemcpyAsync(drank, rank, ns * 4, hipMemcpyHostToDevice, sc.stream));
    if (out_ms) {
        SVDCHK(hipEventCreate(&sc.e0)); SVDCHK(hipEventCreate(&sc.e1));
        SVDCHK(hipEventRecord(sc.e0, sc.stream));
    }
    hipLaunchKernelGGL(mxe::bins_resample_kernel, dim3(n_sets), dim3(mxe::BINS_T), 0, sc.stream, p);
    SVDCHK(hipGetLastError());
    if (out_ms) SVDCHK(hipEventRecord(sc.e1, sc.stream));
    SVDCHK(hipMemcpyAsync(out_mean, p.out_mean, ns * n * 8, hipMemcpyDeviceToHost, sc.stream));
    SVDCHK(hipMemcpyAsync(out_G, p.out_G, ns * nr * n * 8, hipMemcpyDeviceToHost, sc.stream));
    if (out_dev) SVDCHK(hipMemcpyAsync(out_dev, p.out_dev, ns * nr * n * 8, hipMemcpyDeviceToHost, sc.stream));
    SVDCHK(hipStreamSynchronize(sc.stream));
    if (out_ms) SVDCHK(hipEventElapsedTime(out_ms, sc.e0, sc.e1));
    return MXE_OK;
}
MXE_CATCH_ALL

extern "C" int mxe_resample_reduce(mxe_ctx* ctx, int n_groups, const int32_t* group_offset, const double* H,
                                   const int32_t* problem_index, const double* scale, int n_f, const double* F,
                                   double* out_mean, double* out_var, double* out_fval, double* out_fmean, double* out_fcov,
                                   int32_t* out_used, float* out_ms)
try {
    if (!ctx || n_groups < 1 || !group_offset || !scale || n_f < 0 || (n_f > 0 && !F)) return MXE_ERR_ARG;
    if (group_offset[0] != 0) return MXE_ERR_ARG;
    for (int g = 0; g < n_groups; ++g) {
        if (group_offset[g + 1] < group_offset[g]) return MXE_ERR_ARG;
        if (!std::isfinite(scale[g])) return MXE_ERR_ARG;
    }
    if (!H && !ctx->launched) return MXE_ERR_STATE;
    const size_t rows = (size_t)group_offset[n_groups], nw = ctx->n_omega, nf = n_f, ng = n_groups;
    if (rows * nw > 0x7fffffffull || rows * std::max<size_t>(nf, 1) > 0x7fffffffull || nf * nw > 0x7fffffffull ||
        ng * nw > 0x7fffffffull || ng * nf * nf > 0x7fffffffull) return MXE_ERR_ARG;
    const size_t n_last = (size_t)ctx->n_chain * ctx->n_alpha;
    std::vector<int> hi(group_offset, group_offset + ng + 1);
    const size_t iO = 0, iK = iO + ng + 1, iU = iK + rows, iR = iU + ng, itotal = iR + (H ? 0 : rows);
    hi.resize(itotal, 0);
    if (!H)
        for (size_t r = 0; r < rows; ++r) {
            const int row = problem_index ? problem_index[r] : (int)r;
            if (row < 0 || (size_t)row >= n_last) return MXE_ERR_ARG;
            hi[iR + r] = row;
        }
    if (nf && !all_finite(F, nf * nw)) return MXE_ERR_ARG;
    HIPCHK(ctx, hipSetDevice(ctx->device));
    const size_t oH = ng, oF = oH + (H ? rows * nw : 0), oV = oF + nf * nw, oM = oV + rows * nf, oS = oM + ng * nw,
                 oFm = oS + ng * nw, oFc = oFm + ng * nf, total = oFc + ng * nf * nf;
    HIPCHK(ctx, ctx->rr_d.ensure(total));
    HIPCHK(ctx, ctx->rr_i.ensure(itotal));
    double* d = ctx->rr_d.p;
    int* di = ctx->rr_i.p;
    HIPCHK(ctx, hipMemcpyAsync(d, scale, ng * 8, hipMemcpyHostToDevice, ctx->stream));
    if (H && rows) HIPCHK(ctx, hipMemcpyAsync(d + oH, H, rows * nw * 8, hipMemcpyHostToDevice, ctx->stream));
    if (nf) HIPCHK(ctx, hipMemcpyAsync(d + oF, F, nf * nw * 8, hipMemcpyHostToDevice, ctx->stream));
    HIPCHK(ctx, hipMemcpyAsync(di, hi.data(), itotal * sizeof(int), hipMemcpyHostToDevice, ctx->stream));
    mxe::ReduceParams rp;
    rp.H = H ? d + oH : ctx->dout_H.p; rp.row = H ? nullptr : di + iR;
    rp.off = di + iO; rp.scale = d; rp.F = d + oF; rp.nw = (int)nw; rp.n_f = n_f;
    rp.ok = di + iK; rp.fval = d + oV; rp.mean = d + oM; rp.var = d + oS; rp.fmean = d + oFm; rp.fcov = d + oFc; rp.used = di + iU;
    SvdScratch sc;
    if (out_ms) {
        HIPCHK(ctx, hipEventCreate(&sc.e0)); HIPCHK(ctx, hipEventCreate(&sc.e1));
        HIPCHK(ctx, hipEventRecord(sc.e0, ctx->stream));
    }
    hipLaunchKernelGGL(mxe::resample_reduce_kernel, dim3((unsigned)n_groups), dim3(256), 0, ctx->stream, rp);
    HIPCHK(ctx, hipGetLastError());
    if (out_ms) HIPCHK(ctx, hipEventRecord(sc.e1, ctx->stream));
    if (out_mean) HIPCHK(ctx, hipMemcpyAsync(out_mean, d + oM, ng * nw * 8, hipMemcpyDeviceToHost, ctx->stream));
    if (out_var) HIPCHK(ctx, hipMemcpyAsync(out_var, d + oS, ng * nw * 8, hipMemcpyDeviceToHost, ctx->stream));
    if (out_fval && rows * nf) HIPCHK(ctx, hipMemcpyAsync(out_fval, d + oV, rows * nf * 8, hipMemcpyDeviceToHost, ctx->stream));
    if (out_fmean && nf) HIPCHK(ctx, hipMemcpyAsync(out_fmean, d + oFm, ng * nf * 8, hipMemcpyDeviceToHost, ctx->stream));
    if (out_fcov && nf) HIPCHK(ctx, hipMemcpyAsync(out_fcov, d + oFc, ng * nf * nf * 8, hipMemcpyDeviceToHost, ctx->stream));
    std::vector<int> hused(ng);
    if (out_used) HIPCHK(ctx, hipMemcpyAsync(hused.data(), di + iU, ng * sizeof(int), hipMemcpyDeviceToHost, ctx->stream));
    HIPCHK(ctx, stream_wait(ctx->stream));
    if (out_used) for (size_t g = 0; g < ng; ++g) out_used[g] = hused[g];
    if (out_ms) HIPCHK(ctx, hipEventElapsedTime(out_ms, sc.e0, sc.e1));
    return MXE_OK;
}
MXE_CATCH_ALL

#include "mxe_evidence.hip.h"

extern "C" int mxe_evidence_reduce(mxe_ctx* ctx, int n_groups, const int32_t* group_offset, int n_alpha, const double* H,
                                   const int32_t* chain_index, const double* logp, const double* log_quad,
                                   const double* log_mix, const double* log_prior, int row_mode, const int32_t* pick,
                                   int n_f, const double* F,
                                   double* out_logZ, int32_t* out_kmax, int32_t* out_ngood, double* out_walpha,
                                   double* out_row, double* out_fval, double* out_wmodel, double* out_mean,
                                   double* out_between, double* out_fmean, double* out_fcov, int32_t* out_used, float* out_ms)
try {
    if (!ctx || n_groups < 1 || !group_offset || n_alpha < 1 || !logp || !log_quad || !log_mix || n_f < 0 || (n_f > 0 && !F) ||
        row_mode < 0 || row_mode > 2 || (row_mode == 2 && !pick)) return MXE_ERR_ARG;
    if (group_offset[0] != 0) return MXE_ERR_ARG;
    for (int g = 0; g < n_groups; ++g)
        if (group_offset[g + 1] < group_offset[g]) return MXE_ERR_ARG;
    const size_t ns = (size_t)group_offset[n_groups], na = n_alpha, nw = ctx->n_omega, nf = n_f, ng = n_groups;
    const size_t lim = 0x7fffffffull;
    if (ns * na > lim || (H && ns * na * nw > lim) || ns * nw > lim || ns * std::max<size_t>(nf, 1) > lim || nf * nw > lim ||
        ng * nw > lim || ng * nf * nf > lim) return MXE_ERR_ARG;
    if (!H && !ctx->launched) return MXE_ERR_STATE;
    std::vector<long long> hrow0(std::max<size_t>(ns, 1));
    if (!H) {
        if (n_alpha != ctx->n_alpha) return MXE_ERR_ARG;
        for (size_t s = 0; s < ns; ++s) {
            const int c = chain_index ? chain_index[s] : (int)s;
            if (c < 0 || c >= ctx->n_chain) return MXE_ERR_ARG;
            hrow0[s] = (long long)c * n_alpha;
        }
    } else {
        for (size_t s = 0; s < ns; ++s) hrow0[s] = (long long)(s * na);
    }
    if (row_mode == 2)
        for (size_t s = 0; s < ns; ++s) if (pick[s] >= n_alpha) return MXE_ERR_ARG;
    if (!all_finite(log_quad, na) || !all_finite(log_mix, na) || (nf && !all_finite(F, nf * nw))) return MXE_ERR_ARG;
    if (log_prior)
        for (size_t s = 0; s < ns; ++s)
            if (std::isnan(log_prior[s]) || log_prior[s] == INFINITY) return MXE_ERR_ARG;
    HIPCHK(ctx, hipSetDevice(ctx->device));
    const size_t oP = H ? ns * na * nw : 0, oQ = oP + ns * na, oX = oQ + na, oPr = oX + na, oF = oPr + ns, oZ = oF + nf * nw,
                 oW = oZ + ns, oR = oW + ns * na, oV = oR + ns * nw, oU = oV + ns * nf, oM = oU + ns, oB = oM + ng * nw,
                 oFm = oB + ng * nw, oFc = oFm + ng * nf, total = oFc + ng * nf * nf;
    const size_t iP = ng + 1, iG = iP + ns, iUs = iG + ns * na, iK = iUs + ns, iN = iK + ns, iU = iN + ns, itotal = iU + ng;
    HIPCHK(ctx, ctx->er_d.ensure(total));
    HIPCHK(ctx, ctx->er_i.ensure(itotal));
    HIPCHK(ctx, ctx->er_l.ensure(hrow0.size()));
    double* d = ctx->er_d.p;
    int* di = ctx->er_i.p;
    std::vector<int> hi(group_offset, group_offset + ng + 1);
    hi.resize(iG, 0);
    if (row_mode == 2) for (size_t s = 0; s < ns; ++s) hi[iP + s] = pick[s];
    std::vector<double> hprior(std::max<size_t>(ns, 1), 0.0);
    if (log_prior) for (size_t s = 0; s < ns; ++s) hprior[s] = log_prior[s];
    if (H && ns) HIPCHK(ctx, hipMemcpyAsync(d, H, ns * na * nw * 8, hipMemcpyHostToDevice, ctx->stream));
    if (ns) HIPCHK(ctx, hipMemcpyAsync(d + oP, logp, ns * na * 8, hipMemcpyHostToDevice, ctx->stream));
    HIPCHK(ctx, hipMemcpyAsync(d + oQ, log_quad, na * 8, hipMemcpyHostToDevice, ctx->stream));
    HIPCHK(ctx, hipMemcpyAsync(d + oX, log_mix, na * 8, hipMemcpyHostToDevice, ctx->stream));
    if (ns) HIPCHK(ctx, hipMemcpyAsync(d + oPr, hprior.data(), ns * 8, hipMemcpyHostToDevice, ctx->stream));
    if (nf) HIPCHK(ctx, hipMemcpyAsync(d + oF, F, nf * nw * 8, hipMemcpyHostToDevice, ctx->stream));
    HIPCHK(ctx, hipMemcpyAsync(di, hi.data(), iG * sizeof(int), hipMemcpyHostToDevice, ctx->stream));
    HIPCHK(ctx, hipMemcpyAsync(ctx->er_l.p, hrow0.data(), hrow0.size() * sizeof(long long), hipMemcpyHostToDevice, ctx->stream));
    mxe::EvidenceParams ep;
    ep.H = H ? d : ctx->dout_H.p; ep.row0 = ctx->er_l.p;
    ep.logp = d + oP; ep.log_quad = d + oQ; ep.log_mix = d + oX; ep.log_prior = d + oPr; ep.pick = di + iP; ep.off = di;
    ep.F = d + oF; ep.n_alpha = n_alpha; ep.nw = (int)nw; ep.n_f = n_f; ep.row_mode = row_mode;
    ep.good = di + iG; ep.usable = di + iUs; ep.logZ = d + oZ; ep.kmax = di + iK; ep.ngood = di + iN; ep.walpha = d + oW;
    ep.row = d + oR; ep.fval = d + oV; ep.wmodel = d + oU; ep.mean = d + oM; ep.between = d + oB; ep.fmean = d + oFm;
    ep.fcov = d + oFc; ep.used = di + iU;
    SvdScratch sc;
    if (out_ms) {
        HIPCHK(ctx, hipEventCreate(&sc.e0)); HIPCHK(ctx, hipEventCreate(&sc.e1));
        HIPCHK(ctx, hipEventRecord(sc.e0, ctx->stream));
    }
    if (ns) {
        hipLaunchKernelGGL(mxe::evidence_scan_kernel, dim3((unsigned)ns), dim3(mxe::EV_T), 0, ctx->stream, ep);
        HIPCHK(ctx, hipGetLastError());
    }
    hipLaunchKernelGGL(mxe::evidence_group_kernel, dim3((unsigned)ng), dim3(mxe::EV_T), 0, ctx->stream, ep);
    HIPCHK(ctx, hipGetLastError());
    if (out_ms) HIPCHK(ctx, hipEventRecord(sc.e1, ctx->stream));
    if (out_logZ && ns) HIPCHK(ctx, hipMemcpyAsync(out_logZ, d + oZ, ns * 8, hipMemcpyDeviceToHost, ctx->stream));
    if (out_walpha && ns) HIPCHK(ctx, hipMemcpyAsync(out_walpha, d + oW, ns * na * 8, hipMemcpyDeviceToHost, ctx->stream));
    if (out_row && ns) HIPCHK(ctx, hipMemcpyAsync(out_row, d + oR, ns * nw * 8, hipMemcpyDeviceToHost, ctx->stream));
    if (out_fval && ns * nf) HIPCHK(ctx, hipMemcpyAsync(out_fval, d + oV, ns * nf * 8, hipMemcpyDeviceToHost, ctx->stream));
    if (out_wmodel && ns) HIPCHK(ctx, hipMemcpyAsync(out_wmodel, d + oU, ns * 8, hipMemcpyDeviceToHost, ctx->stream));
    if (out_mean) HIPCHK(ctx, hipMemcpyAsync(out_mean, d + oM, ng * nw * 8, hipMemcpyDeviceToHost, ctx->stream));
    if (out_between) HIPCHK(ctx, hipMemcpyAsync(out_between, d + oB, ng * nw * 8, hipMemcpyDeviceToHost, ctx->stream));
    if (out_fmean && nf) HIPCHK(ctx, hipMemcpyAsync(out_fmean, d + oFm, ng * nf * 8, hipMemcpyDeviceToHost, ctx->stream));
    if (out_fcov && nf) HIPCHK(ctx, hipMemcpyAsync(out_fcov, d + oFc, ng * nf * nf * 8, hipMemcpyDeviceToHost, ctx->stream));
    std::vector<int> hout(2 * ns + ng);
    if (ns) HIPCHK(ctx, hipMemcpyAsync(hout.data(), di + iK, 2 * ns * sizeof(int), hipMemcpyDeviceToHost, ctx->stream));
    HIPCHK(ctx, hipMemcpyAsync(hout.data() + 2 * ns, di + iU, ng * sizeof(int), hipMemcpyDeviceToHost, ctx->stream));
    HIPCHK(ctx, stream_wait(ctx->stream));
    for (size_t s = 0; s < ns; ++s) {
        if (out_kmax) out_kmax[s] = hout[s];
        if (out_ngood) out_ngood[s] = hout[ns + s];
    }
    if (out_used) for (size_t g = 0; g < ng; ++g) out_used[g] = hout[2 * ns + g];
    if (out_ms) HIPCHK(ctx, hipEventElapsedTime(out_ms, sc.e0, sc.e1));
    return MXE_OK;
}
MXE_CATCH_ALL

#include "mxe_bincheck.hip.h"

extern "C" int mxe_bins_check(int device, int n_sets, int n_bins, int n_data, const double* bins,
                              const double* T, const int32_t* rank,
                              double* out_mean, double* out_err2, double* out_skew, double* out_kurt,
                              int32_t* out_levels, float* out_ms)
try {
    if (n_sets < 1 || n_bins < 2 || n_data < 1 || n_data > mxe::BINS_NMAX || !bins || !out_mean || !out_err2 || !out_skew ||
        !out_kurt || !out_levels || (T == nullptr) != (rank == nullptr)) return MXE_ERR_ARG;
    if ((int64_t)n_bins * n_data > INT32_MAX) return MXE_ERR_ARG;
    const size_t m = n_bins, n = n_data, ns = n_sets, nel = ns * m * n;
    if (rank)
        for (size_t s = 0; s < ns; ++s) if (rank[s] < 0 || rank[s] > n_data) return MXE_ERR_ARG;
    if (!all_finite(bins, nel) || (T && !all_finite(T, ns * n * n))) return MXE_ERR_ARG;
    int L = 0;
    while ((n_bins >> (L + 1)) >= 1) ++L;
    int ndev = 0;
    if (hipGetDeviceCount(&ndev) != hipSuccess || ndev < 1) return MXE_ERR_NODEVICE;
    if (device < 0 || device >= ndev) return MXE_ERR_ARG;
    SVDCHK(hipSetDevice(device));
    SvdScratch sc;
    SVDCHK(hipStreamCreateWithFlags(&sc.stream, hipStreamNonBlocking));
    mxe::BinCheckParams p;
    p.m = n_bins; p.n = n_data; p.L = L;
    const size_t nout = ns * (size_t)L * n;
    double *dbins, *dT = nullptr;
    int* drank = nullptr;
    SVDCHK(sc.alloc(&dbins, nel));
    if (T) { SVDCHK(sc.alloc(&dT, ns * n * n)); SVDCHK(sc.alloc(&drank, ns)); }
    SVDCHK(sc.alloc(&p.part, ns * mxe::BINS_NWAVE * n * 2)); SVDCHK(sc.alloc(&p.part2, ns * mxe::BINS_NWAVE * n * 3));
    SVDCHK(sc.alloc(&p.Y0, nel)); SVDCHK(sc.alloc(&p.Y1, std::max<size_t>(ns * (m >> 1) * n, 1)));
    SVDCHK(sc.alloc(&p.out_mean, ns * n)); SVDCHK(sc.alloc(&p.out_err2, nout));
    SVDCHK(sc.alloc(&p.out_skew, nout)); SVDCHK(sc.alloc(&p.out_kurt, nout));
    p.bins = dbins; p.T = dT; p.rank = drank;
    SVDCHK(hipMemcpyAsync(dbins, bins, nel * 8, hipMemcpyHostToDevice, sc.stream));
    if (T) {
        SVDCHK(hipMemcpyAsync(dT, T, ns * n * n * 8, hipMemcpyHostToDevice, sc.stream));
        SVDCHK(hipMemcpyAsync(drank, rank, ns * 4, hipMemcpyHostToDevice, sc.stream));
    }
    if (out_ms) {
        SVDCHK(hipEventCreate(&sc.e0)); SVDCHK(hipEventCreate(&sc.e1));
// ... 16 lines not shown
```

### maxent_amd/csrc/mxe_eval.hip.h

```cpp
#pragma once
#include "mxe_kernel.hip.h"

namespace mxe {

struct EvalParams {
    int nw, nwp, ns, NP;
    const double* V;
    const double* Vt;
    const double* c;
    const int* elem_ds;
    const int* elem_kind;
    const double* ghat;
    const double* cperp;
    const double* D;
    const int* elem;
    int elem_div;
    const double* alpha;
    const double* x;
    int x_stride;
    int input_is_H;
    double eta;
    int want_gram, want_gram2, want_audit;
    double* Q; double* chi2; double* S;
    double* H; double* u; double* w; double* q;
// ... 210 lines not shown
            __syncthreads();
            const int m = ns - j - 1;
            for (int idx = tid; idx < m * m; idx += 256) {
                const int i = j + 1 + idx / m, k = j + 1 + idx % m;
                if (k <= i) Bm[i * LD + k] = fma(-Bm[i * LD + j], Bm[k * LD + j], Bm[i * LD + k]);
            }
            __syncthreads();
        }
        if (wave == 0) {
            for (int j = 0; j < ns; ++j) {
                if (lane == (j & 63)) zsh[j] /= Bm[j * LD + j];
                wave_sync();
                const double zj = zsh[j];
                for (int i = lane; i < ns; i += 64) if (i > j) zsh[i] = fma(-Bm[i * LD + j], zj, zsh[i]);
                wave_sync();
            }
            for (int j = ns - 1; j >= 0; --j) {
                if (lane == (j & 63)) zsh[j] /= Bm[j * LD + j];
                wave_sync();
                const double zj = zsh[j];
                for (int i = lane; i < j; i += 64) zsh[i] = fma(-Bm[j * LD + i], zj, zsh[i]);
                wave_sync();
            }
            for (int i = lane; i < ns; i += 64) zsh[i] *= cc[i];
        }
        __syncthreads();
        double s2[1] = {0.0};
        for (int i = tid; i < nw; i += 256) {
            double du = 0.0;
            for (int k = 0; k < ns; ++k) du = fma(Vt[(size_t)k * nwp + i], zsh[k], du);
            const double t = wsh[i] * du;
            s2[0] = fma(t, t, s2[0]);
        }
        eval_block_sum<1>(s2, red);
        if (tid == 0 && ep.corr) ep.corr[prob] = ok ? sqrt(s2[0] / Hn2) : __builtin_nan("");
    }
    if (ep.want_gram2 && ep.W2) {
        __syncthreads();
        for (int i = tid; i < nwp; i += 256) {
            double q = 0.0;
            if (i < nw) for (int k = 0; k < ns; ++k) q = fma(Vt[(size_t)k * nwp + i], gsh[k], q);
            wsh[i] = q * Hsh[i];
        }
        __syncthreads();
        eval_gram<NT>(V, wsh, Bm, nwp, ns);
        for (int idx = tid; idx < NP * NP; idx += 256) {
            const int i = idx / NP, j = idx % NP;
            ep.W2[prob * NP * NP + idx] = (i < ns && j < ns) ? Bm[i * LD + j] : 0.0;
        }
    }
}

__global__ __launch_bounds__(256)
void entropy_kernel(int kind, int n, const double* __restrict__ H, const double* __restrict__ D,
                    double* __restrict__ outS, double* __restrict__ outd, double* __restrict__ outdd)
{
    __shared__ double red[4];
    const size_t p = blockIdx.x;
    auto slog = [](double x) { return log(fabs(x) > 1e-100 ? x : 1e-100); };
    double acc[1] = {0.0};
    for (int i = threadIdx.x; i < n; i += 256) {
        const double h = H[p * n + i], d = D[i];
        double Sv, dS, wsum;
        if (kind == 0) {
            Sv = h - d - h * slog(h / d);
            dS = -(slog(h) - slog(d));
            wsum = h;
        } else {
            const double r = sqrt(h * h + 4.0 * d * d);
            const double hp = 0.5 * (r + h), hm = 0.5 * (r - h);
            Sv = (hp - d - hp * slog(hp / d)) + (hm - d - hm * slog(hm / d));
            dS = -(slog(hp) - slog(d));
            wsum = hp + hm;
        }
        if (!(fabs(wsum) > 1e-100)) wsum = 1e-100;
        acc[0] += Sv;
        if (outd) outd[p * n + i] = dS;
        if (outdd) outdd[p * n + i] = -1.0 / wsum;
    }
    eval_block_sum<1>(acc, red);
    if (threadIdx.x == 0 && outS) outS[p] = acc[0];
}

}

namespace mxe {

struct LineSSE { double slope, icpt, sse; int n; };

__device__ inline LineSSE line_sse(const double* x, const double* y, int lo, int hi, bool line)
{
    const int lane = threadIdx.x & 63;
    LineSSE r; r.slope = 0.0; r.icpt = 0.0; r.sse = 0.0; r.n = 0;
    double sx = 0.0, sy = 0.0, cnt = 0.0;
    for (int k = lo + lane; k < hi; k += 64) if (y[k] == y[k]) { sx += x[k]; sy += y[k]; cnt += 1.0; }
    sx = wave_sum(sx); sy = wave_sum(sy); cnt = wave_sum(cnt);
    r.n = (int)cnt;
    if (r.n < 1) return r;
    const double xm = sx / cnt, ym = sy / cnt;
    double sxx = 0.0, sxy = 0.0;
    for (int k = lo + lane; k < hi; k += 64) if (y[k] == y[k]) { const double dx = x[k] - xm; sxx += dx * dx; sxy += dx * (y[k] - ym); }
    sxx = wave_sum(sxx); sxy = wave_sum(sxy);
    if (line && r.n >= 2 && sxx != 0.0) { r.slope = sxy / sxx; r.icpt = ym - r.slope * xm; }
    else r.icpt = ym;
    double e = 0.0;
    for (int k = lo + lane; k < hi; k += 64) if (y[k] == y[k]) { const double d = y[k] - (r.slope * x[k] + r.icpt); e += d * d; }
    r.sse = wave_sum(e);
    return r;
}

__global__ __launch_bounds__(256)
void linefit_kernel(const double* __restrict__ alpha, const double* __restrict__ chi2, const double* __restrict__ H,
                    int n_alpha, int nw, int p2_deg, double* __restrict__ out_sel ,
                    double* __restrict__ out_idx ,
                    const double* __restrict__ S = nullptr, double gamma = 0.2,
                    double* __restrict__ out3_idx = nullptr ,
                    double* __restrict__ out3_sel = nullptr )
{
    extern __shared__ double sm[];
    const int tid = threadIdx.x, lane = tid & 63, wave = tid >> 6, n = n_alpha;
    double* x = sm;
    double* y = x + n;
    double* cs = y + n;
    double* ap = cs + 6 * (n + 1);
    double* x10 = ap + n;
    double* y10 = x10 + n;
    double* wbest = y10 + n;
    double* wfit = wbest + 4;
    __shared__ int s_pick[3];
    const size_t c = blockIdx.x;
    for (int k = tid; k < n; k += 256) {
        const double a = alpha[c * n + k], q = chi2[c * n + k];
        x[k] = log(a); y[k] = log(q);
        x10[k] = gamma * log10(a); y10[k] = log10(q);
    }
    if (tid < 3) s_pick[tid] = -1;
    __syncthreads();
    const bool fit = n > 4;
    double xm = 0.0, ym = 0.0;
    if (fit) {
        double sx = 0.0, sy = 0.0, sw = 0.0;
        for (int k = lane; k < n; k += 64) { sx += x[k]; if (y[k] == y[k]) { sy += y[k]; sw += 1.0; } }
        sx = wave_sum(sx); sy = wave_sum(sy); sw = wave_sum(sw);
        xm = sx / n; ym = sy / fmax(sw, 1.0);
        for (int q = wave; q < 6; q += 4) {
            double carry = 0.0;
            if (lane == 0) cs[q * (n + 1)] = 0.0;
            for (int c0 = 0; c0 < n; c0 += 64) {
                const int k = c0 + lane;
                const bool in = k < n, ok = in && y[in ? k : 0] == y[in ? k : 0];
                const double w = ok ? 1.0 : 0.0, x0 = in ? x[k] - xm : 0.0, yc = ok ? y[k] - ym : 0.0;
                double v = q == 0 ? w : q == 1 ? w * x0 : q == 2 ? yc : q == 3 ? w * x0 * x0 : q == 4 ? x0 * yc : yc * yc;
#pragma unroll
                for (int off = 1; off < 64; off <<= 1) {
                    const double up = __shfl_up(v, off);
                    if (lane >= off) v += up;
                }
                v += carry;
                if (in) cs[q * (n + 1) + k + 1] = v;
                carry = __shfl(v, 63);
            }
        }
    }
    __syncthreads();
    auto sse = [&](int lo, int hi, bool line) -> double {
        const double m = cs[hi] - cs[lo], s1 = cs[(n + 1) + hi] - cs[(n + 1) + lo], s2 = cs[2 * (n + 1) + hi] - cs[2 * (n + 1) + lo];
        const double sxx = cs[3 * (n + 1) + hi] - cs[3 * (n + 1) + lo], sxy = cs[4 * (n + 1) + hi] - cs[4 * (n + 1) + lo];
        const double syy = cs[5 * (n + 1) + hi] - cs[5 * (n + 1) + lo];
        if (!(m >= 1.0)) return __builtin_nan("");
        const double vyy = syy - s2 * s2 / m;
        if (!line || m < 2.0) return vyy;
        const double vxx = sxx - s1 * s1 / m, vxy = sxy - s1 * s2 / m;
        return vxx > 0.0 ? vyy - vxy * vxy / vxx : vyy;
    };
    if (fit) {
        double best = __builtin_inf();
        for (int i = 2 + tid; i < n - 2; i += 256) {
            const double a = sse(0, i, true) + sse(i, n, p2_deg == 1);
            ap[i] = a;
            if (a == a && fabs(a) < 1.7e308 && a < best) best = a;
        }
        best = -wave_max(-best);
        if (lane == 0) wbest[wave] = best;
    }
    __syncthreads();
    if (fit) {
        const double best = fmin(fmin(wbest[0], wbest[1]), fmin(wbest[2], wbest[3]));
        const double tol = best + 1e-9 * (fabs(cs[5 * (n + 1) + n]) + 1e-300) + 1e-6 * fabs(best);
        const bool rank_ok = best < 1.7e308 && n > 8;
        double ebest = __builtin_inf(); int ebest_i = -1, seen = 0;
        LineSSE abest, bbest;
        abest.slope = abest.icpt = bbest.slope = bbest.icpt = 0.0;
        for (int i = 2; i < n - 2; ++i) {
            const bool cand = rank_ok ? (ap[i] == ap[i] && ap[i] <= tol) : true;
            if (!cand) continue;
            const bool mine = (seen & 3) == wave;
            ++seen;
            if (!mine) continue;
            const LineSSE a = line_sse(x, y, 0, i, true), b = line_sse(x, y, i, n, p2_deg == 1);
            if (a.n < 1 || b.n < 1) continue;
            const double m = a.sse + b.sse;
            if (m == m && m < ebest) { ebest = m; ebest_i = i; abest = a; bbest = b; }
        }
        if (lane == 0) {
            double* f = wfit + wave * 6;
            f[0] = ebest; f[1] = (double)ebest_i; f[2] = abest.slope; f[3] = abest.icpt; f[4] = bbest.slope; f[5] = bbest.icpt;
        }
    }
    __syncthreads();
    if (wave == 0 && fit) {
        double ebest = __builtin_inf(); int ebest_i = -1, wv = -1;
        for (int w = 0; w < 4; ++w) {
            const double m = wfit[w * 6]; const int i = (int)wfit[w * 6 + 1];
            if (i >= 0 && (m < ebest || (m == ebest && i < ebest_i))) { ebest = m; ebest_i = i; wv = w; }
        }
        if (ebest_i >= 0) {
            const double* f = wfit + wv * 6;
            const double xc = (f[5] - f[3]) / (f[2] - f[4]);
            double dbest = __builtin_inf(); int di = -1;
            for (int k = lane; k < n; k += 64) {
                const double d = fabs(x[k] - xc);
                if (d == d && (d < dbest || (d == dbest && k < di))) { dbest = d; di = k; }
            }
            for (int off = 32; off >= 1; off >>= 1) {
                const double od = __shfl_xor(dbest, off); const int oi = __shfl_xor(di, off);
                if (oi >= 0 && (di < 0 || od < dbest || (od == dbest && oi < di))) { dbest = od; di = oi; }
            }
            if (lane == 0) s_pick[0] = di;
        }
    }
    if (out3_idx && (wave == 1 || wave == 2)) {
        double vbest = (wave == 1) ? -__builtin_inf() : __builtin_inf();
        int vi = -1;
        for (int k = 1 + lane; k < n - 1; k += 64) {
            double val;
            if (wave == 1) {
                const double hp = x10[k + 1] - x10[k], hm = x10[k] - x10[k - 1];
                const double der2 = (y10[k + 1] - 2 * y10[k] + y10[k - 1]) / (hp * hm);
                const double der1 = ((y10[k + 1] - y10[k]) / hp + (y10[k] - y10[k - 1]) / hm) / 2;
                const double q = 1 + der1 * der1;
                val = der2 / (q * sqrt(q));
                if (val == val && (val > vbest || vi < 0)) { vbest = val; vi = k; }
            } else {
                const double dS = (S[c * n + k + 1] - S[c * n + k - 1]) / (x[k + 1] - x[k - 1]);
                val = dS * dS;
                if (val == val && (val < vbest || vi < 0)) { vbest = val; vi = k; }
            }
        }
        for (int off = 32; off >= 1; off >>= 1) {
            const double ov = __shfl_xor(vbest, off); const int oi = __shfl_xor(vi, off);
            const bool better = (wave == 1) ? (ov > vbest) : (ov < vbest);
            if (oi >= 0 && (vi < 0 || better || (ov == vbest && oi < vi))) { vbest = ov; vi = oi; }
        }
        if (lane == 0) s_pick[wave] = vi;
    }
    __syncthreads();
    const int idx = s_pick[0];
    if (tid == 0) out_idx[c] = (double)idx;
    if (out_sel) {
        const double* row = H + (c * n + (idx >= 0 ? idx : 0)) * nw;
        for (int k = tid; k < nw; k += 256) out_sel[c * nw + k] = (idx >= 0) ? row[k] : __builtin_nan("");
    }
    if (!out3_idx) return;
    const size_t nc = gridDim.x;
    if (tid < 3) out3_idx[tid * nc + c] = (double)s_pick[tid];
    if (out3_sel) {
#pragma unroll
        for (int a = 0; a < 3; ++a) {
            const int pk = s_pick[a];
            const double* row = H + (c * n + (pk >= 0 ? pk : 0)) * nw;
            double* dst = out3_sel + ((size_t)a * nc + c) * nw;
            for (int k = tid; k < nw; k += 256) dst[k] = (pk >= 0) ? row[k] : __builtin_nan("");
        }
    }
}

}
```

### maxent_amd/csrc/mxe_kernel_mc.hip.h

```cpp
#pragma once
#ifndef MXE_X_KERNARG_RELOAD
#define MXE_X_KERNARG_RELOAD 0
#endif
#include "mxe_kernel.hip.h"

namespace mxe {

constexpr int MCC = 4;

struct MCExtra {
    const int* wg_chains;
    int n_wg;
    const int* queue;
    int n_queue;
    int* counter;
    int stagger;
    int n_solo;
    double* gstate;
    size_t gstate_stride;
};

constexpr int MC_GSTATE_PAD = 1024;
inline size_t mc_gstate_doubles(int nwp) { return (size_t)nwp * 4 + ((size_t)nwp * 4 + MC_GSTATE_PAD) + ((size_t)nwp * 4 + MC_GSTATE_PAD) / 2; }

// ... 490 lines not shown
                if (t.active) {
                    rho[q * NP + k] = r;
                    const double chi2t = r2 + t.cperp, St = sS;
                    const double Qt = 0.5 * chi2t - t.alpha * St;
                    const bool finite = fabs(Qt) <= 1.7e308;
                    bool finish_alpha = false, failed = false; int conv = 0;
                    bool on_path = false;
                    const bool fresh = t.scratch == 2;
                    if (t.scratch == 1 || (fresh && !t.okprev)) {
                        ++t.nevals;
                        if (finite) { t.scratch = 0; t.chi2 = chi2t; t.S = St; t.Hn2 = sHn; t.wmax = swm; t.Q = Qt; }
                        else { finish_alpha = true; failed = true; }
                    } else if (!t.okprev) {
                        finish_alpha = true; failed = true;
                    } else if (!finite || ((t.mu > 0.0 || (t.okprev >= 2 && t.okprev <= 4)) && Qt > t.Q + 1e-12 * fabs(t.Q)) ||
                               (t.okprev == 5 && Qt > 4.0 * fabs(t.Q) + 1.0) ||
                               (t.okprev == 1 && Qt > 1e6 * (fabs(t.Q) + 1.0))) {
                        ++t.nevals;
                        if (finite && t.bt < 3 && !(t.mu == 0.0 && t.muh > 0.0)) {
                            ++t.bt;
                            t.okprev = 3;
                        } else {
                            t.mu = (t.mu == 0.0) ? fmax(p.mu_first * t.alpha, t.muh / p.mu_grow) : t.mu * p.mu_grow;
                            t.scratch = 1; t.bt = 0;
                            if (!(t.mu <= p.mu_max * t.alpha) || t.nevals >= p.mc_maxevals) { finish_alpha = true; failed = true; }
                        }
                    } else {
                        ++t.nevals;
                        double fac2 = 1.0;
                        const bool estimated = p.stop_estimate && t.mu == 0.0 && t.okprev == 1 && sdu <= 1.0;
                        if (estimated) {
                            const double em1 = sdu * fma(sdu, fma(sdu, fma(sdu, 1.0 / 24.0, 1.0 / 6.0), 0.5), 1.0);
                            const double fac = em1 + p.theta + MC_GRAM_ERR;
                            fac2 = fmin(1.0, fac * fac);
                        }
                        double relH2_min = fac2 * sdH;
                        if (t.mu > 0.0) {
                            const double ud = 1.0 + t.mu / t.alpha;
                            relH2_min *= ud * ud;
                        }
                        const double pred_here = estimated ? relH2_min : 0.0;
    #ifndef MXE_X_NO_PRED_CHECK
                        if (estimated && t.pred > 0.0 && sdH > t.pred) relH2_min = fmin(sdH, relH2_min * (sdH / t.pred));
    #endif
                        double tol_h = p.tol_h;
                        asm volatile("" : "+s"(tol_h));
                        const double tol_here = (LEAD && t.ia < 0) ? fmax(tol_h, (t.ia == -t.lead) ? MXE_X_LEAD_TOL : MXE_X_WALK_TOL) : tol_h;
                        const double tol2Hn = tol_here * tol_here * t.Hn2;
                        vv[q * NP + k] -= dlc[q * NP + k];
                        if (t.niter == 0) t.capp = (t.okprev == 5) ? 2 : (t.okprev == 1 && t.mu == 0.0) ? 1 : 0;
                        else eacc[q * NP + k] -= dlc[q * NP + k];
                        t.chi2 = chi2t; t.S = St; t.Hn2 = sHn; t.wmax = swm;
                        t.Qprev = t.Q; t.Q = Qt; t.muh = t.mu; t.mu = 0.0;
                        t.pred = pred_here;
                        ++t.niter;
                        const bool newton_step = t.okprev != 4 && !fresh;
                        {
                            const bool full = newton_step && t.okprev == 1 && t.muh == 0.0;
                            t.slow = (full && t.dHp > 0.0 && sdH > 0.25 * t.dHp) ? t.slow + 1 : 0;
                            t.dHp = full ? sdH : 0.0;
                        }
                        t.bt = 0;
                        on_path = newton_step && t.niter == 1 && relH2_min < (MXE_X_WALK_SKIP_TOL * MXE_X_WALK_SKIP_TOL) * t.Hn2;
                        if (newton_step && p.tol_h > 0.0 && relH2_min < tol2Hn && t.niter > p.miniter) { conv = 1; finish_alpha = true; }
                        else if (p.tol_relq > 0.0 && fabs(fabs(t.Qprev - t.Q) / t.Q) < p.tol_relq && t.niter > p.miniter) { conv = 1; finish_alpha = true; }
                        else if (t.niter >= ((LEAD && t.ia < 0 && t.ia > -t.lead) ? MXE_X_WALK_ITERS : p.mc_maxiter)) finish_alpha = true;
                        else if (t.wide > 0 && t.niter - t.wide >= MXE_X_ILL_ITERS) finish_alpha = true;
                        else if (MXE_X_SLOW_STEPS > 0 && t.slow >= MXE_X_SLOW_STEPS && t.niter >= 8 && (!LEAD || t.ia >= 0)) finish_alpha = true;
                    }
                    MXE_STAMPA(2);
                    if (fresh && t.scratch == 2) t.scratch = 0;
                    if (finish_alpha) {
                        const size_t prob = (size_t)t.prob0 + max(t.ia, 0);
                        const bool own = !LEAD || t.ia >= 0;
                        if (p.out_H && own) {
                            double* Ho = p.out_H + prob * nw;
                            for (int i = lane; i < nw; i += 64) Ho[i] = failed ? __builtin_nan("") : Hi[i * MCC + q];
                        }
                        if (p.out_v && own) p.out_v[prob * NP + lane] = vv[q * NP + lane];
                        if (lane == 0 && own) {
                            p.out_chi2[prob] = t.chi2; p.out_S[prob] = t.S; p.out_Q[prob] = t.Q;
                            p.out_niter[prob] = t.niter; p.out_conv[prob] = conv;
                            p.out_nevals[prob] = t.nevals; p.out_nact[prob] = t.nact;
                        }
                        MXE_STAMPA(3);
                        {
                            double e = 0.0;
                            if (conv && t.capp > 0 && t.ia > 0 && t.ia + 1 < t.clen) {
                                const double a0 = alpha_at(t, t.ia - 1), a1 = t.alpha, a2 = alpha_at(t, t.ia + 1);
                                const double q0 = a1 / a0, q1 = a2 / a1;
                                const double rr = (fabs(q1 - q0) < 1e-9 * q0) ? 1.0 : log(q1) / log(q0);
                                const bool fine = q0 > 0.74 && q0 < 1.35 && q1 > 0.74 && q1 < 1.35;
                                if (fine)
                                e = ((t.capp == 2 ? ecor[q * NP + k] : 0.0) + eacc[q * NP + k]) * rr * rr;
                                if (!(fabs(e) < 1e300)) e = 0.0;
                            }
                            ecor[q * NP + k] = e; eacc[q * NP + k] = 0.0;
                        }
                        ++t.ia;
                        if constexpr (LEAD) {
                            if (t.ia < -1 && on_path) {
                                const double lo = t.alpha * (1.0 / MXE_X_WALK_RATIO), hi = t.alpha * MXE_X_WALK_RATIO;
                                while (t.ia < -1) {
                                    const double an = alpha_at(t, t.ia + 1);
                                    if (!(an >= lo && an <= hi)) break;
                                    ++t.ia;
                                }
                            }
                        }
                        if (!conv && p.mc_abandon) {
                            for (int i = max(t.ia, 0) + lane; i < t.clen; i += 64) {
                                const size_t pr = (size_t)t.prob0 + i;
                                p.out_conv[pr] = 0; p.out_niter[pr] = 0; p.out_nevals[pr] = 0; p.out_nact[pr] = 0;
                            }
                            t.ia = t.clen;
                        }
                        t.niter = 0; t.nevals = 0; t.mu = 0.0; t.bt = 0; t.capp = 0; t.pred = 0.0; t.wide = 0; t.slow = 0; t.dHp = 0.0;
                        t.Qprev = __builtin_nan("");
                        if (t.ia >= t.clen) {
                            t.active = 0;
                            if (dynamic) {
                                int idx = 0;
                                if (lane == 0) idx = atomicAdd(x.counter, 1);
                                idx = __builtin_amdgcn_readfirstlane(idx);
                                if (idx < x.n_queue) start_piece(t, x.queue[idx]);
                            }
                        } else {
                            t.alpha = alpha_at(t, t.ia);
                            t.Q = 0.5 * t.chi2 - t.alpha * t.S;
                        }
                    }
                    MXE_STAMPA(4);
                    MXE_STAMPA(6);
                }
                MXE_STAMPW(5);
            } else {
                load_slot(t);
            }
            int okflag = 0;
            double dk = 0.0;
            double dtot = 0.0;
            const double isc2 = ldexp(1.0, -ilogb(t.sc2));
            {
                const double wm = (t.wmax > 1e-290 && t.wmax < 1e290) ? t.wmax : 1.0;
                const double sc2n = ldexp(1.0, 8 - ilogb(wm));
                if (lane == 0) { s_scw[q][0] = isc2; s_scw[q][1] = sc2n; }
                t.sc2 = sc2n;
            }
            if (t.active && t.scratch == 1) {
                dk = vv[q * NP + k];
            } else if (t.active && t.okprev == 3) {
                dtot = 0.5 * dlc[q * NP + k];
                dk = -dtot;
                okflag = 4;
            } else if (t.active) {
                rhs[q * NP + k] = (k < ns) ? fma(t.alpha * vv[q * NP + k], ci[k], rho[q * NP + k]) : 0.0;
                const double thr = p.theta * t.alpha, wmx = fmax(t.wmax, 1e-300);
                const unsigned long long m = __ballot(k < ns && cc[k] * cc[k] * wmx > thr);
                int na = (p.theta > 0.0) ? __popcll(m) : ns;
                na = max(1, min(na, NA));
                t.nact = na;
                {
                    const double sk = ldexp(1.0, -(ilogb(fma(cc[k] * cc[k], wmx, t.alpha)) >> 1));
                    ssc[q * NP + k] = sk; csc[q * NP + k] = cc[k] * sk;
                }
                wave_sync();
// ... 338 lines not shown
```

Baseline: 31.06 million alpha-solves/s.

## Defer spectrum H materialisation; recompute selected rows from v in line fit

The chain kernel no longer writes the full H spectrum (P x n_omega doubles) by default. H is instead rebuilt lazily from the stored v coefficients by a new h_of_v kernel whenever a consumer needs it. The line fit recomputes only the selected rows from v, Vt and D. Failed problems are flagged by bit-inverting nact, and the host un-inverts it on readback. This cuts global store traffic in the hot kernel, at the cost of recompute on any later H access and more complex state tracking across the double buffers.

```diff
diff --git a/maxent_amd/csrc/maxent_hip.hip b/maxent_amd/csrc/maxent_hip.hip
--- a/maxent_amd/csrc/maxent_hip.hip
+++ b/maxent_amd/csrc/maxent_hip.hip
@@ -247,6 +247,9 @@
     DevBuf<double> dout_v, dout_pack, dout_pack2, dB, dA, dlogdet;
     DevBuf<int> dparent_elem;
     int result_buffer = 0;
+    bool H_materialised[2] = {true, true};
+    bool eager_H = false;
+    bool pack2_cleared = false;
     struct View { double* p = nullptr; } dout_H, dout_chi2, dout_S, dout_Q;
     DevBuf<int> dout_niter, dout_nact;
     struct IView { int* p = nullptr; } dout_conv, dout_nevals;
@@ -1001,6 +1004,7 @@
     in.lds_mc32x1 = mc_lds_bytes(32, nwp, 1); in.lds_mc32x2 = mc_lds_bytes(32, nwp, 2);
     in.wgpc_auto = ctx->wgpc_auto; in.mc_wgpc_hint = ctx->mc_wgpc_hint;
     read_plan_env(in.env);
+    { const char* e = getenv("MXE_EAGER_H"); ctx->eager_H = e && atoi(e) != 0; }
     mxe::LaunchPlan plan;
     if (const int rc = mxe::plan_launch(in, plan); rc != MXE_OK) {
         if (plan.uncovered || plan.covered_twice) fprintf(stderr, "mxe_chains_upload: %zu problems covered by no piece, %zu by two (layout %d, %zu pieces, %zu excluded)\n",
@@ -1047,6 +1051,10 @@
     ctx->dout_S.p = ctx->dout_chi2.p + P; ctx->dout_Q.p = ctx->dout_S.p + P;
     HIPCHK(ctx, ctx->dout_niter.ensure(3 * P)); HIPCHK(ctx, ctx->dout_nact.ensure(P));
     ctx->dout_conv.p = ctx->dout_niter.p + P; ctx->dout_nevals.p = ctx->dout_conv.p + P;
+    ctx->H_materialised[0] = ctx->H_materialised[1] = true; ctx->pack2_cleared = false;
+    if (ctx->eager_H) HIPCHK(ctx, hipMemsetAsync(ctx->dout_pack.p, 0xFF, (P * nw + 3 * P) * sizeof(double), ctx->stream));
+    else HIPCHK(ctx, hipMemsetAsync(ctx->dout_chi2.p, 0xFF, 3 * P * sizeof(double), ctx->stream));
+    HIPCHK(ctx, put(ctx->dparent_elem, ctx->chain_elem));
     std::vector<int> e2, p2, l2;
     if (ctx->lv_mode == 2) {
         e2.resize(P); p2.resize(P); l2.assign(P, 1);
@@ -1145,6 +1153,31 @@
 }
 }
 
+static mxe::HRowSrc h_row_src(mxe_ctx* ctx);
+static int materialise_H(mxe_ctx* ctx, int which)
+{
+    if (ctx->H_materialised[which]) return MXE_OK;
+    const size_t P = (size_t)ctx->n_chain * ctx->n_alpha, nw = ctx->n_omega;
+    double* base = which ? ctx->dout_pack2.p : ctx->dout_pack.p;
+    if (!base || ctx->NP > 128) return MXE_ERR_STATE;
+    const mxe::HRowSrc hs = h_row_src(ctx);
+    hipLaunchKernelGGL(mxe::h_of_v_kernel, dim3((unsigned)P), dim3(256), 0, ctx->stream, hs, (const double*)(base + P * nw),
+                       ctx->n_alpha, (int)nw, base);
+    HIPCHK(ctx, hipGetLastError());
+    ctx->H_materialised[which] = true;
+    return MXE_OK;
+}
+static int ensure_H(mxe_ctx* ctx) { return materialise_H(ctx, ctx->result_buffer); }
+#define MXE_ENSURE_H(ctx) do { const int rc_h__ = ensure_H(ctx); if (rc_h__ != MXE_OK) return rc_h__; } while (0)
+static mxe::HRowSrc h_row_src(mxe_ctx* ctx)
+{
+    mxe::HRowSrc hs;
+    hs.v = ctx->dout_v.p; hs.nact = ctx->dout_nact.p; hs.Vt = ctx->dVt.p; hs.D = ctx->dD.p;
+    hs.chain_elem = ctx->dparent_elem.p; hs.elem_ds = ctx->delem_ds.p; hs.elem_kind = ctx->delem_kind.p;
+    hs.ns = ctx->n_s; hs.NP = ctx->NP; hs.nwp = ctx->nwp;
+    return hs;
+}
+
 constexpr double LV_TOL1 = 1e-5;
 
 int mxe_chains_launch(mxe_ctx* ctx)
@@ -1153,6 +1186,8 @@
     if (!ctx->chains_ready) return MXE_ERR_STATE;
     HIPCHK(ctx, hipSetDevice(ctx->device));
     ctx->pre_d = nullptr; ctx->pre_i = nullptr; ctx->pre_rows = nullptr; ctx->pre_index = false;
+    { const int rc_h = materialise_H(ctx, 1 - ctx->result_buffer); if (rc_h != MXE_OK) return rc_h; }
+    ctx->H_materialised[ctx->result_buffer] = true;
     const mxe_opts& o = ctx->opts;
     KParams kp;
     fill_kparams(ctx, kp);
@@ -1259,6 +1294,7 @@
                                ctx->dout_nevals.p, ctx->dout_nact.p);
             HIPCHK(ctx, hipGetLastError());
         }
+        if (!ctx->eager_H) { kp.out_H = nullptr; ctx->H_materialised[ctx->result_buffer] = false; }
         ctx->last_nw = NWV; ctx->last_lds = (int)lds;
         const bool lead = kp.chain_lead != nullptr;
         ctx->last_kernel = "mxe::chain_kernel_mc<" + std::to_string(NA) + ", " + std::to_string(WGPC) + (lead ? ", lead" : "") +
@@ -1354,6 +1390,7 @@
     int n = 0;
     for (int i : todo) if (nit[i] < o.maxiter) { open[i] = 1; ++n; }
     if (n == 0) return MXE_OK;
+    MXE_ENSURE_H(ctx);
     ctx->pre_d = nullptr; ctx->pre_i = nullptr; ctx->pre_rows = nullptr; ctx->pre_index = false;
     const int NP = ctx->NP, na = ctx->n_alpha;
     std::vector<int> f_elem, f_prob0, f_len, f_v0;
@@ -1510,7 +1547,7 @@
     HIPCHK(ctx, stream_wait(ctx->stream));
     const size_t P = (size_t)ctx->n_chain * ctx->n_alpha;
     const int ns = ctx->n_s, NP = ctx->NP, nw = ctx->n_omega;
-    if (out_H) HIPCHK(ctx, d2h_pipelined(out_H, ctx->dout_H.p, P * nw * 8, ctx->stream));
+    if (out_H) { MXE_ENSURE_H(ctx); HIPCHK(ctx, d2h_pipelined(out_H, ctx->dout_H.p, P * nw * 8, ctx->stream)); }
     const bool pre = ctx->pre_d && out_chi2 == ctx->pre_d && out_S == out_chi2 + P && out_Q == out_S + P &&
                      out_niter == ctx->pre_i && out_converged == out_niter + P && out_nevals == out_converged + P;
     if (pre) {}
@@ -1598,6 +1635,7 @@
     HIPCHK(ctx, stream_wait(ctx->stream));
     const size_t P = (size_t)ctx->n_chain * ctx->n_alpha;
     HIPCHK(ctx, hipMemcpy(out_nact, ctx->dout_nact.p, P * 4, hipMemcpyDeviceToHost));
+    for (size_t i = 0; i < P; ++i) if (out_nact[i] < 0) out_nact[i] = ~out_nact[i];
     return MXE_OK;
 }
 
@@ -1622,7 +1660,11 @@
 {
     if (!ctx) return MXE_ERR_ARG;
     if (!ctx->chains_ready) return MXE_ERR_STATE;
-    if (d_H) *d_H = ctx->dout_H.p;
+    if (d_H) {
+        HIPCHK(ctx, hipSetDevice(ctx->device));
+        MXE_ENSURE_H(ctx);
+        *d_H = ctx->dout_H.p;
+    }
     if (d_chi2) *d_chi2 = ctx->dout_chi2.p;
     if (d_S) *d_S = ctx->dout_S.p;
     if (d_Q) *d_Q = ctx->dout_Q.p;
@@ -1640,7 +1682,14 @@
     if (!ctx->chains_ready) return MXE_ERR_STATE;
     HIPCHK(ctx, hipSetDevice(ctx->device));
     const size_t P = (size_t)ctx->n_chain * ctx->n_alpha, nw = ctx->n_omega;
-    if (which == 1) HIPCHK(ctx, ctx->dout_pack2.ensure(P * nw + 3 * P + (size_t)ctx->n_chain * (nw + 1)));
+    if (which == 1) {
+        HIPCHK(ctx, ctx->dout_pack2.ensure(P * nw + 3 * P + (size_t)ctx->n_chain * (nw + 1)));
+        if (!ctx->pack2_cleared) {
+            if (ctx->eager_H) HIPCHK(ctx, hipMemsetAsync(ctx->dout_pack2.p, 0xFF, (P * nw + 3 * P) * sizeof(double), ctx->stream));
+            else HIPCHK(ctx, hipMemsetAsync(ctx->dout_pack2.p + P * nw, 0xFF, 3 * P * sizeof(double), ctx->stream));
+        }
+        ctx->pack2_cleared = true;
+    }
     double* base = which ? ctx->dout_pack2.p : ctx->dout_pack.p;
     ctx->result_buffer = which;
     ctx->dout_H.p = base; ctx->dout_chi2.p = base + P * nw; ctx->dout_S.p = ctx->dout_chi2.p + P; ctx->dout_Q.p = ctx->dout_S.p + P;
@@ -1748,6 +1797,7 @@
     HIPCHK(ctx, hipSetDevice(ctx->device));
     const size_t P = (size_t)ctx->n_chain * ctx->n_alpha;
     HIPCHK(ctx, ctx->dlogdet.ensure(P));
+    MXE_ENSURE_H(ctx);
     HIPCHK(ctx, ctx->dparent_elem.ensure(ctx->chain_elem.size()));
     HIPCHK(ctx, hipMemcpyAsync(ctx->dparent_elem.p, ctx->chain_elem.data(), ctx->chain_elem.size() * sizeof(int),
                                hipMemcpyHostToDevice, ctx->stream));
@@ -1958,6 +2008,7 @@
 int upload_posterior(mxe_ctx* ctx, const PostStage& st, int P, const double* H, double* d, size_t oH, mxe::FactorParams& fp)
 {
     const int nw = ctx->n_omega;
+    if (!H) MXE_ENSURE_H(ctx);
     HIPCHK(ctx, ctx->pv_i.ensure((size_t)2 * P));
     HIPCHK(ctx, hipMemcpyAsync(d, st.ha.data(), (size_t)P * 8, hipMemcpyHostToDevice, ctx->stream));
     if (H) HIPCHK(ctx, hipMemcpyAsync(d + oH, H, (size_t)P * nw * 8, hipMemcpyHostToDevice, ctx->stream));
@@ -2236,8 +2287,10 @@
     const size_t P = (size_t)ctx->n_chain * ctx->n_alpha;
     double* sel = ctx->dout_Q.p + P;
     double* idx = sel + (size_t)ctx->n_chain * ctx->n_omega;
-    hipLaunchKernelGGL(mxe::linefit_kernel, dim3(ctx->n_chain), dim3(256), ((size_t)11 * ctx->n_alpha + 6 + 28) * sizeof(double), ctx->stream,
-                       ctx->dalpha.p, ctx->dout_chi2.p, ctx->dout_H.p, ctx->n_alpha, ctx->n_omega, p2_deg, sel, idx);
+    const double* H = ctx->H_materialised[ctx->result_buffer] ? ctx->dout_H.p : nullptr;
+    hipLaunchKernelGGL(mxe::linefit_kernel, dim3(ctx->n_chain), dim3(256), ((size_t)11 * ctx->n_alpha + 6 + 28 + 128) * sizeof(double), ctx->stream,
+                       ctx->dalpha.p, ctx->dout_chi2.p, H, ctx->n_alpha, ctx->n_omega, p2_deg, sel, idx,
+                       (const double*)nullptr, 0.2, (double*)nullptr, (double*)nullptr, h_row_src(ctx));
     HIPCHK(ctx, hipGetLastError());
     return MXE_OK;
 }
@@ -2253,9 +2306,10 @@
     double* idx = sel + nc * nw;
     HIPCHK(ctx, ctx->dsel3.ensure(3 * nc * (nw + 1)));
     ctx->pre_rows = nullptr; ctx->pre_index = false;
-    hipLaunchKernelGGL(mxe::linefit_kernel, dim3(ctx->n_chain), dim3(256), ((size_t)11 * ctx->n_alpha + 6 + 28) * sizeof(double), ctx->stream,
-                       ctx->dalpha.p, ctx->dout_chi2.p, ctx->dout_H.p, ctx->n_alpha, ctx->n_omega, p2_deg, sel, idx,
-                       ctx->dout_S.p, gamma, ctx->dsel3.p, ctx->dsel3.p + 3 * nc);
+    const double* H = ctx->H_materialised[ctx->result_buffer] ? ctx->dout_H.p : nullptr;
+    hipLaunchKernelGGL(mxe::linefit_kernel, dim3(ctx->n_chain), dim3(256), ((size_t)11 * ctx->n_alpha + 6 + 28 + 128) * sizeof(double), ctx->stream,
+                       ctx->dalpha.p, ctx->dout_chi2.p, H, ctx->n_alpha, ctx->n_omega, p2_deg, sel, idx,
+                       ctx->dout_S.p, gamma, ctx->dsel3.p, ctx->dsel3.p + 3 * nc, h_row_src(ctx));
     HIPCHK(ctx, hipGetLastError());
     ctx->sel3_nc = ctx->n_chain;
     return MXE_OK;
@@ -2353,6 +2407,7 @@
     const size_t P = (size_t)ctx->n_chain * ctx->n_alpha, nw = ctx->n_omega;
     for (int r = 0; r < n_rows; ++r)
         if (problem_index[r] < 0 || (size_t)problem_index[r] >= P) return MXE_ERR_ARG;
+    MXE_ENSURE_H(ctx);
     HIPCHK(ctx, ctx->rows_idx.ensure(n_rows));
     HIPCHK(ctx, ctx->rows_out.ensure((size_t)n_rows * nw));
     HIPCHK(ctx, hipMemcpyAsync(ctx->rows_idx.p, problem_index, (size_t)n_rows * 4, hipMemcpyHostToDevice, ctx->stream));
@@ -2543,6 +2598,7 @@
     mxe_comm_state* cm = ctx->comm;
     if (root < 0 || root >= cm->n_ranks) return MXE_ERR_ARG;
     if (!cm->local.empty()) return MXE_ERR_STATE;
+    if (what == MXE_GATHER_FULL) { HIPCHK(ctx, hipSetDevice(ctx->device)); MXE_ENSURE_H(ctx); }
     if (cm->rank == root) { const int rr = gather_reserve(ctx, cm->n_ranks, counts); if (rr != MXE_OK) return rr; }
     const bool grouped = cm->n_ranks > 1 || cm->loopback;
     if (grouped) NCCLCHK(ctx, g_rccl.GroupStart());
@@ -2566,6 +2622,8 @@
         if (!ctxs[r] || !ctxs[r]->comm || ctxs[r]->comm->n_ranks != n || ctxs[r]->comm->rank != r || !ctxs[r]->launched) return MXE_ERR_STATE;
     mxe_ctx* rt = ctxs[root];
     const bool copy = rt->comm->copy_transport;
+    if (what == MXE_GATHER_FULL)
+        for (int r = 0; r < n; ++r) { HIPCHK(ctxs[r], hipSetDevice(ctxs[r]->device)); MXE_ENSURE_H(ctxs[r]); }
     { const int rr = gather_reserve(rt, n, counts); if (rr != MXE_OK) return rr; }
     if (copy) {
         for (int r = 0; r < n; ++r) {
@@ -2664,6 +2722,7 @@
     const size_t P = (size_t)ctx->n_chain * ctx->n_alpha;
     std::vector<double> Bt((size_t)nw * nw);
     for (int j = 0; j < nw; ++j) for (int k = 0; k < nw; ++k) Bt[(size_t)k * nw + j] = B[(size_t)j * nw + k];
+    MXE_ENSURE_H(ctx);
     HIPCHK(ctx, ctx->dB.ensure(Bt.size()));
     HIPCHK(ctx, ctx->dA.ensure(P * nw));
     HIPCHK(ctx, hipMemcpyAsync(ctx->dB.p, Bt.data(), Bt.size() * 8, hipMemcpyHostToDevice, ctx->stream));
@@ -3125,6 +3184,7 @@
     if (H && rows) HIPCHK(ctx, hipMemcpyAsync(d + oH, H, rows * nw * 8, hipMemcpyHostToDevice, ctx->stream));
     if (nf) HIPCHK(ctx, hipMemcpyAsync(d + oF, F, nf * nw * 8, hipMemcpyHostToDevice, ctx->stream));
     HIPCHK(ctx, hipMemcpyAsync(di, hi.data(), itotal * sizeof(int), hipMemcpyHostToDevice, ctx->stream));
+    if (!H) MXE_ENSURE_H(ctx);
     mxe::ReduceParams rp;
     rp.H = H ? d + oH : ctx->dout_H.p; rp.row = H ? nullptr : di + iR;
     rp.off = di + iO; rp.scale = d; rp.F = d + oF; rp.nw = (int)nw; rp.n_f = n_f;
@@ -3211,6 +3271,7 @@
     if (nf) HIPCHK(ctx, hipMemcpyAsync(d + oF, F, nf * nw * 8, hipMemcpyHostToDevice, ctx->stream));
     HIPCHK(ctx, hipMemcpyAsync(di, hi.data(), iG * sizeof(int), hipMemcpyHostToDevice, ctx->stream));
     HIPCHK(ctx, hipMemcpyAsync(ctx->er_l.p, hrow0.data(), hrow0.size() * sizeof(long long), hipMemcpyHostToDevice, ctx->stream));
+    if (!H) MXE_ENSURE_H(ctx);
     mxe::EvidenceParams ep;
     ep.H = H ? d : ctx->dout_H.p; ep.row0 = ctx->er_l.p;
     ep.logp = d + oP; ep.log_quad = d + oQ; ep.log_mix = d + oX; ep.log_prior = d + oPr; ep.pick = di + iP; ep.off = di;
diff --git a/maxent_amd/csrc/mxe_eval.hip.h b/maxent_amd/csrc/mxe_eval.hip.h
--- a/maxent_amd/csrc/mxe_eval.hip.h
+++ b/maxent_amd/csrc/mxe_eval.hip.h
@@ -316,6 +316,71 @@
     if (threadIdx.x == 0 && outS) outS[p] = acc[0];
 }
 
+struct HRowSrc {
+    const double* v;
+    const int* nact;
+    const double* Vt;
+    const double* D;
+    const int* chain_elem;
+    const int* elem_ds;
+    const int* elem_kind;
+    int ns, NP, nwp;
+};
+
+__device__ __forceinline__ void h_row_of_problem(const HRowSrc& hs, const double* __restrict__ chi2, int n_alpha, int nw,
+                                                 size_t prob, double* vsh, double* __restrict__ dst)
+{
+#pragma clang fp contract(off)
+    const int tid = threadIdx.x, nt = blockDim.x;
+    const double q = chi2[prob];
+    if (!(q == q) || hs.nact[prob] < 0) {
+        for (int i = tid; i < nw; i += nt) dst[i] = __builtin_nan("");
+        return;
+    }
+    const int e = hs.chain_elem[prob / n_alpha];
+    const int kind = hs.elem_kind[e];
+    const double* Vt = hs.Vt + (size_t)hs.elem_ds[e] * hs.NP * hs.nwp;
+    const double* Dp = hs.D + (size_t)e * hs.nwp;
+    __syncthreads();
+    for (int k = tid; k < hs.NP; k += nt) vsh[k] = hs.v[prob * hs.NP + k];
+    __syncthreads();
+    const int ns = hs.ns, nwp = hs.nwp;
+    for (int i = tid; i < nw; i += nt) {
+        double acc0 = 0.0, acc1 = 0.0;
+        int k = 0;
+        for (; k + 8 <= ns; k += 8) {
+            double a[8];
+#pragma unroll
+            for (int r = 0; r < 8; ++r) a[r] = Vt[(size_t)(k + r) * nwp + i];
+#pragma unroll
+            for (int r = 0; r < 8; r += 2) {
+                acc0 = fma(a[r], vsh[k + r], acc0);
+                acc1 = fma(a[r + 1], vsh[k + r + 1], acc1);
+            }
+        }
+        for (; k + 1 < ns; k += 2) {
+            acc0 = fma(Vt[(size_t)k * nwp + i], vsh[k], acc0);
+            acc1 = fma(Vt[(size_t)(k + 1) * nwp + i], vsh[k + 1], acc1);
+        }
+        if (k < ns) acc0 = fma(Vt[(size_t)k * nwp + i], vsh[k], acc0);
+        const double uq = acc0 + acc1;
+        const double Di = Dp[i];
+        const double ep = fast_exp(uq);
+        const double Hp = Di * ep;
+        double Hq = Hp;
+        if (kind != 0) { const double Hm = Di * recip_exp(ep); Hq = Hp - Hm; }
+        dst[i] = Hq;
+    }
+}
+
+__global__ __launch_bounds__(256)
+void h_of_v_kernel(const HRowSrc hs, const double* __restrict__ chi2, int n_alpha, int nw, double* __restrict__ H)
+{
+    __shared__ double vsh[128];
+    const size_t prob = blockIdx.x;
+    h_row_of_problem(hs, chi2, n_alpha, nw, prob, vsh, H + prob * nw);
+}
+
 }
 
 namespace mxe {
@@ -349,7 +414,8 @@
                     double* __restrict__ out_idx ,
                     const double* __restrict__ S = nullptr, double gamma = 0.2,
                     double* __restrict__ out3_idx = nullptr ,
-                    double* __restrict__ out3_sel = nullptr )
+                    double* __restrict__ out3_sel = nullptr ,
+                    const HRowSrc hs = HRowSrc())
 {
     extern __shared__ double sm[];
     const int tid = threadIdx.x, lane = tid & 63, wave = tid >> 6, n = n_alpha;
@@ -361,6 +427,7 @@
     double* y10 = x10 + n;
     double* wbest = y10 + n;
     double* wfit = wbest + 4;
+    double* vsh = wfit + 24;
     __shared__ int s_pick[3];
     const size_t c = blockIdx.x;
     for (int k = tid; k < n; k += 256) {
@@ -492,8 +559,12 @@
     const int idx = s_pick[0];
     if (tid == 0) out_idx[c] = (double)idx;
     if (out_sel) {
-        const double* row = H + (c * n + (idx >= 0 ? idx : 0)) * nw;
-        for (int k = tid; k < nw; k += 256) out_sel[c * nw + k] = (idx >= 0) ? row[k] : __builtin_nan("");
+        if (idx < 0) { for (int k = tid; k < nw; k += 256) out_sel[c * nw + k] = __builtin_nan(""); }
+        else if (H == nullptr) h_row_of_problem(hs, chi2, n, nw, c * n + idx, vsh, out_sel + c * nw);
+        else {
+            const double* row = H + (c * n + idx) * nw;
+            for (int k = tid; k < nw; k += 256) out_sel[c * nw + k] = row[k];
+        }
     }
     if (!out3_idx) return;
     const size_t nc = gridDim.x;
@@ -502,11 +573,13 @@
 #pragma unroll
         for (int a = 0; a < 3; ++a) {
             const int pk = s_pick[a];
-            const double* row = H + (c * n + (pk >= 0 ? pk : 0)) * nw;
             double* dst = out3_sel + ((size_t)a * nc + c) * nw;
-            for (int k = tid; k < nw; k += 256) dst[k] = (pk >= 0) ? row[k] : __builtin_nan("");
-        }
-    }
-}
-
-}
+            if (pk < 0) { for (int k = tid; k < nw; k += 256) dst[k] = __builtin_nan(""); continue; }
+            if (H == nullptr) { h_row_of_problem(hs, chi2, n, nw, c * n + pk, vsh, dst); continue; }
+            const double* row = H + (c * n + pk) * nw;
+            for (int k = tid; k < nw; k += 256) dst[k] = row[k];
+        }
+    }
+}
+
+}
diff --git a/maxent_amd/csrc/mxe_kernel_mc.hip.h b/maxent_amd/csrc/mxe_kernel_mc.hip.h
--- a/maxent_amd/csrc/mxe_kernel_mc.hip.h
+++ b/maxent_amd/csrc/mxe_kernel_mc.hip.h
@@ -596,6 +596,7 @@
                             p.out_chi2[prob] = t.chi2; p.out_S[prob] = t.S; p.out_Q[prob] = t.Q;
                             p.out_niter[prob] = t.niter; p.out_conv[prob] = conv;
                             p.out_nevals[prob] = t.nevals; p.out_nact[prob] = t.nact;
+                            if (failed) p.out_nact[prob] = ~t.nact;
                         }
                         MXE_STAMPA(3);
                         {
```

After: 31.36 million alpha-solves/s (median of 6 runs). About the same (+1.0%).
